# JJKK1313/DiTreeOnlinePlanner

Measured on AMD Instinct MI355X. Metric: candidate tree-expansions/sec (carmaze, H=32), higher is better.
Workload: dtype f16x3; 1 GPU; cfgs/carmaze.yaml + fm_policy flow sampler (K=1), batch=1024 candidates per GPU, H=32 (4 chunks x 8 steps), boxes.csv 20x20, 1024-node tree snapshot, seeded random weights; batch_per_gpu=1024, global_batch=1024, edge_length=32, action_horizon=8, pred_horizon=64, flow_steps=1, tree_nodes=1024, parallelism=candidates sharded x1

## Files before the change

ditreeonlineplanner_amd/csrc/conv_tiles.hip:

```cpp
#include <type_traits>

#include "denoise_device.h"

static thread_local bool g_dn_dry_run = false;
void denoise_set_dry_run(bool on) { g_dn_dry_run = on; }
bool denoise_dry_run() { return g_dn_dry_run; }

template <int PREC>
__device__ __forceinline__ void gemm_epilogue(const ConvGemmParams& p, f32x16_t (&acc)[2][4], char* smem, int tm, int tn,
                                              int tid, int lane, int r5, int h, int wm, int wn,
                                              long long out_extra_bytes = 0) {

  constexpr int ET = PREC == 2 ? 1 : 0;
  float satm = 0.0f;
  const int c_l = wn * 128 + 4 * r5;
  const int n0 = tn * 256 + c_l;
  const bool n_ok = n0 < p.N;
  float bias4[4] = {0.f, 0.f, 0.f, 0.f};
  if (p.bias != nullptr && n_ok) {
    f32x4_t t = *(const f32x4_t*)(p.bias + n0);
#pragma unroll
    for (int j = 0; j < 4; ++j) bias4[j] = t[j];
  }
#pragma unroll
  for (int mb = 0; mb < 2; ++mb)
#pragma unroll
    for (int j = 0; j < 4; ++j)
#pragma unroll
      for (int i = 0; i < 16; ++i) {
        if constexpr (PREC == 2) acc[mb][j][i] = fmaf(acc[mb][j][i], p.w_scale, bias4[j]);
        else acc[mb][j][i] += bias4[j];
      }

  int blk_b[4], blk_l[4];
#pragma unroll
  for (int blk = 0; blk < 4; ++blk) {
    const int m0 = tm * 256 + wm * 64 + (blk >> 1) * 32 + (blk & 1) * 16;
    const int b = m0 / p.L;
    blk_b[blk] = b;
    blk_l[blk] = m0 - b * p.L;
  }

  if (p.mode >= MODE_GN_MISH) {
    float* s_sum = (float*)smem;
    float* s_sq = s_sum + 64;
    if (tid < 128) s_sum[tid] = 0.0f;
    const f32x4_t gam = *(const f32x4_t*)(p.gamma + n0);
    const f32x4_t bet = *(const f32x4_t*)(p.beta + n0);
    f32x4_t film_s[4], film_b[4];
    if (p.mode == MODE_GN_MISH_FILM) {
#pragma unroll
      for (int blk = 0; blk < 4; ++blk) {
        const float* fr = p.film + (long long)blk_b[blk] * p.film_ld + p.film_off + n0;
        film_s[blk] = *(const f32x4_t*)fr;
        film_b[blk] = *(const f32x4_t*)(fr + p.N);
      }
    }
    short4_t resv[2][8];
    auto fetch_res = [&](int blk, short4_t (&dst)[8]) {
#pragma unroll
      for (int i = 0; i < 8; ++i) {
        const int rofs = (i & 3) + 8 * (i >> 2) + 4 * h;
        const long long rrow = (long long)blk_b[blk] * p.res_Lp + blk_l[blk] + rofs + p.res_off;
        dst[i] = *(const short4_t*)((const char*)p.Res + (rrow * p.ldres + n0) * 2);
      }
    };
    const bool res_bf16 = (PREC != 1) && p.mode == MODE_GN_MISH_RES;
    if (res_bf16) fetch_res(0, resv[0]);
    __syncthreads();
    const int spt = 256 / p.L;
    const int gi = c_l / p.group_ch;
    const bool wide = p.group_ch >= 128;
    int slot[4];
#pragma unroll
    for (int blk = 0; blk < 4; ++blk) slot[blk] = blk_b[blk] - tm * spt;
    const float inv_cnt = 1.0f / (float)(p.group_ch * p.L);
    const bool ordered = p.L >= 128 || (p.group_ch == 256 && p.L >= 32);
    const bool adder = lane == 0 || (!wide && lane == 16);
    const int ocell = ((wm * 2 + wn) * 4 + gi) * 2;
    auto put = [&](float* cell, float (&t)[4]) {
      if (ordered) {
        if (p.L >= 64) { t[0] = (t[0] + t[1]) + (t[2] + t[3]); t[2] = 0.0f; }
        else { t[0] += t[1]; t[2] += t[3]; }
        if (adder) { cell[ocell] = t[0]; cell[ocell + 1] = t[2]; }
      } else if (adder) {
#pragma unroll
        for (int blk = 0; blk < 4; ++blk) atomicAdd(&cell[slot[blk] * 4 + gi], t[blk]);
      }
    };
    auto get = [&](const float* cell, float (&t)[4]) {
      if (!ordered) {
#pragma unroll
        for (int blk = 0; blk < 4; ++blk) t[blk] = cell[slot[blk] * 4 + gi];
        return;
      }
#pragma unroll
      for (int blk = 0; blk < 4; blk += 2) {
        const int r0 = slot[blk] * p.L;
        const int w0 = r0 >> 6, nw = p.L >= 64 ? p.L >> 6 : 1, sub = (r0 >> 5) & 1;
        float v = 0.0f;
        for (int w = w0; w < w0 + nw; ++w) {
          v += cell[((w * 2 + 0) * 4 + gi) * 2 + sub];
          v += cell[((w * 2 + 1) * 4 + gi) * 2 + sub];
        }
        t[blk] = v; t[blk + 1] = v;
      }
    };
    float mean[4], rstd[4];
    if constexpr (PREC != 1) {
      float ps[4], pq[4];
#pragma unroll
      for (int blk = 0; blk < 4; ++blk) {
        float s = 0.f, q = 0.f;
#pragma unroll
        for (int j = 0; j < 4; ++j)
#pragma unroll
          for (int i = 0; i < 8; ++i) {
            const float v = acc[blk >> 1][j][(blk & 1) * 8 + i];
            s += v;
            q = fmaf(v, v, q);
          }
        s += __shfl_xor(s, 1); q += __shfl_xor(q, 1);
        s += __shfl_xor(s, 2); q += __shfl_xor(q, 2);
        s += __shfl_xor(s, 4); q += __shfl_xor(q, 4);
        s += __shfl_xor(s, 8); q += __shfl_xor(q, 8);
        s += __shfl_xor(s, 32); q += __shfl_xor(q, 32);
        if (wide) { s += __shfl_xor(s, 16); q += __shfl_xor(q, 16); }
        ps[blk] = s; pq[blk] = q;
      }
      put(s_sum, ps);
      put(s_sq, pq);
      __syncthreads();
      get(s_sum, ps);
      get(s_sq, pq);
#pragma unroll
      for (int blk = 0; blk < 4; ++blk) {
        mean[blk] = ps[blk] * inv_cnt;
        const float var = fmaxf(pq[blk] * inv_cnt - mean[blk] * mean[blk], 0.0f);
        rstd[blk] = rsqrtf(var + p.eps);
      }
    } else {
    {
      float ps[4];
#pragma unroll
      for (int blk = 0; blk < 4; ++blk) {
        float s = 0.f;
#pragma unroll
        for (int j = 0; j < 4; ++j)
#pragma unroll
          for (int i = 0; i < 8; ++i) s += acc[blk >> 1][j][(blk & 1) * 8 + i];
        ps[blk] = s;
      }
#pragma unroll
      for (int blk = 0; blk < 4; ++blk) {
        float s = ps[blk];
        s += __shfl_xor(s, 1); s += __shfl_xor(s, 2); s += __shfl_xor(s, 4); s += __shfl_xor(s, 8);
        s += __shfl_xor(s, 32);
        if (wide) s += __shfl_xor(s, 16);
        ps[blk] = s;
      }
      put(s_sum, ps);
      __syncthreads();
      get(s_sum, ps);
#pragma unroll
      for (int blk = 0; blk < 4; ++blk) mean[blk] = ps[blk] * inv_cnt;
    }
    {
      float ps[4];
#pragma unroll
      for (int blk = 0; blk < 4; ++blk) {
        float s = 0.f;
#pragma unroll
        for (int j = 0; j < 4; ++j)
#pragma unroll
          for (int i = 0; i < 8; ++i) {
            float d = acc[blk >> 1][j][(blk & 1) * 8 + i] - mean[blk];
            s += d * d;
          }
        s += __shfl_xor(s, 1); s += __shfl_xor(s, 2); s += __shfl_xor(s, 4); s += __shfl_xor(s, 8);
        s += __shfl_xor(s, 32);
        if (wide) s += __shfl_xor(s, 16);
        ps[blk] = s;
      }
      put(s_sq, ps);
      __syncthreads();
      get(s_sq, ps);
#pragma unroll
      for (int blk = 0; blk < 4; ++blk) rstd[blk] = rsqrtf(ps[blk] * inv_cnt + p.eps);
    }

    }

#pragma unroll
    for (int blk = 0; blk < 4; ++blk) {
      if (res_bf16 && blk < 3) fetch_res(blk + 1, resv[(blk + 1) & 1]);
      f32x4_t fs = {1.f, 1.f, 1.f, 1.f}, fb = {0.f, 0.f, 0.f, 0.f};
      if (p.mode == MODE_GN_MISH_FILM) { fs = film_s[blk]; fb = film_b[blk]; }
      float ga[4], be[4];
#pragma unroll
      for (int j = 0; j < 4; ++j) { ga[j] = gam[j] * rstd[blk]; be[j] = bet[j] - mean[blk] * ga[j]; }
#pragma unroll
      for (int i = 0; i < 8; ++i) {
        const int ii = (blk & 1) * 8 + i;
        const int rofs = (i & 3) + 8 * (i >> 2) + 4 * h;
        const int b = blk_b[blk], l = blk_l[blk] + rofs;
        float v[4];
#pragma unroll
        for (int j = 0; j < 4; ++j) v[j] = mish_f<PREC == 1 ? 1 : 0>(acc[blk >> 1][j][ii] * ga[j] + be[j]) * fs[j] + fb[j];
        if (p.mode == MODE_GN_MISH_RES) {
          if constexpr (PREC != 1) {
            const short4_t rv = resv[blk & 1][i];
#pragma unroll
            for (int j = 0; j < 4; ++j) v[j] += e2f<ET>((unsigned short)rv[j]);
          } else {
            const long long rrow = (long long)b * p.res_Lp + l + p.res_off;
            const f32x4_t rv = *(const f32x4_t*)((const char*)p.Res + (rrow * p.ldres + n0) * 4);
#pragma unroll
            for (int j = 0; j < 4; ++j) v[j] += rv[j];
          }
        }
        const long long orow = (long long)b * p.out_Lp + (long long)l * p.out_stride + p.out_off;
        const long long oidx = orow * p.ldc + p.out_coff + n0;
        if constexpr (PREC == 1) {
          const f32x4_t o = {v[0], v[1], v[2], v[3]};
          *(f32x4_t*)((char*)p.Out + out_extra_bytes + oidx * 4) = o;
        } else {
          short4_t o;
          if constexpr (ET == 1) { sat_see2(satm, v[0], v[1]); sat_see2(satm, v[2], v[3]); }
#pragma unroll
          for (int j = 0; j < 4; ++j) o[j] = (short)f2e<ET>(v[j]);
          *(short4_t*)((char*)p.Out + out_extra_bytes + oidx * 2) = o;
        }
      }
    }
    if constexpr (ET == 1) sat_flush(p.sat, satm);
    return;
  }

#pragma unroll
  for (int blk = 0; blk < 4; ++blk) {
#pragma unroll
    for (int i = 0; i < 8; ++i) {
      const int ii = (blk & 1) * 8 + i;
      const int rofs = (i & 3) + 8 * (i >> 2) + 4 * h;
      const int m = tm * 256 + wm * 64 + (blk >> 1) * 32 + (blk & 1) * 16 + rofs;
      if (m >= p.M || !n_ok) continue;
      int b = blk_b[blk], l = blk_l[blk] + rofs;
      if ((p.L & 15) != 0) { b = m / p.L; l = m - b * p.L; }
      const long long orow = (long long)b * p.out_Lp + (long long)l * p.out_stride + p.out_off;
      const long long oidx = orow * p.ldc + p.out_coff + n0;
      if (p.out_f32 || PREC == 1) {
        const f32x4_t o = {acc[blk >> 1][0][ii], acc[blk >> 1][1][ii], acc[blk >> 1][2][ii], acc[blk >> 1][3][ii]};
        *(f32x4_t*)((char*)p.Out + out_extra_bytes + oidx * 4) = o;
      } else {
        short4_t o;
        if constexpr (ET == 1) { sat_see2(satm, acc[blk >> 1][0][ii], acc[blk >> 1][1][ii]); sat_see2(satm, acc[blk >> 1][2][ii], acc[blk >> 1][3][ii]); }
#pragma unroll
        for (int j = 0; j < 4; ++j) o[j] = (short)f2e<ET>(acc[blk >> 1][j][ii]);
        *(short4_t*)((char*)p.Out + out_extra_bytes + oidx * 2) = o;
      }
    }
  }
  if constexpr (ET == 1) sat_flush(p.sat, satm);
}

template <int PREC, bool C2D = false>
__global__ void __launch_bounds__(512, 2) conv_gemm_kernel(ConvGemmParams p) {
  constexpr int ES = (PREC == 1) ? 4 : 2;
  constexpr int ET = PREC == 2 ? 1 : 0;
  constexpr int EK = 128 / ES;
  constexpr int EPS = 16 / ES;
  extern __shared__ __attribute__((aligned(16))) char smem[];

  const int tid = threadIdx.x, lane = tid & 63, w = tid >> 6;
  const int r5 = lane & 31, h = lane >> 5;
  const int wm = w >> 1, wn = w & 1;
  const int ntn = (p.N + 255) >> 8;
  const int ntm = (p.M + 255) >> 8;
  const int tile = xcd_remap(blockIdx.x, ntm * ntn);
  const int tm = tile / ntn, tn = tile - tm * ntn;
  const int K = p.taps * p.Cin;
  const int kpt = p.Cin / EK;
  int nk = K / EK;
  int k_first = 0;
  long long out_extra = 0;
  if constexpr (C2D) {
    if (p.splitk > 1) {
      const int per = (nk + p.splitk - 1) / p.splitk;
      k_first = blockIdx.y * per;
      nk = min(nk - k_first, per);
      out_extra = (long long)blockIdx.y * p.slab_stride * 4;
    }
  }

  const char* Abase = (const char*)p.A;
  const char* Wbase = (const char*)p.W;
  long long aoff[4], boff[4];
#pragma unroll
  for (int q = 0; q < 4; ++q) {
    const int r = (w * 4 + q) * 8 + (lane >> 3);
    const int sw = (r >> 1) & 7;
    const int slot = (lane & 7) ^ sw;
    int m = tm * 256 + r;
    m = m < p.M ? m : p.M - 1;
    const int b = m / p.L, l = m - b * p.L;
    aoff[q] = (((long long)b * p.in_Lp + (long long)l * p.in_stride + p.in_off) * p.lda + slot * EPS) * ES;
    const int c = (r & 128) + 4 * (r & 31) + ((r >> 5) & 3);
    boff[q] = (((long long)(tn * 256 + c)) * K + slot * EPS) * ES;
  }
  const char* pa[4];
  const char* pb[4];
#pragma unroll
  for (int q = 0; q < 4; ++q) {
    pa[q] = Abase + aoff[q];
    pb[q] = Wbase + boff[q] + (long long)k_first * 128;
  }
  int kin = C2D ? (k_first % kpt) : 0;
  const long long a_tap_jump = ((long long)p.lda - (long long)p.Cin + EK) * ES;
  const char* c2_base[4];
  int c2_ih0[4], c2_iw0[4], c2_slot[4];
  int c2_tap = C2D ? (k_first / kpt) : 0;
  if constexpr (C2D) {
#pragma unroll
    for (int q = 0; q < 4; ++q) {
      const int r = (w * 4 + q) * 8 + (lane >> 3);
      int m = tm * 256 + r;
      m = m < p.M ? m : p.M - 1;
      const int b = m / p.c2_OHW, rem = m - b * p.c2_OHW;
      const int oh = rem / p.c2_OW, ow = rem - oh * p.c2_OW;
      c2_base[q] = Abase + (long long)b * p.c2_H * p.c2_W * p.Cin * ES;
      c2_ih0[q] = oh * p.c2_stride - p.c2_pad;
      c2_iw0[q] = ow * p.c2_stride - p.c2_pad;
      c2_slot[q] = ((lane & 7) ^ ((r >> 1) & 7)) * 16;
    }
  }
  auto c2_point = [&]() {
    const int kh = p.c2_kh[c2_tap], kw = p.c2_kw[c2_tap];
#pragma unroll
    for (int q = 0; q < 4; ++q) {
      const int ih = c2_ih0[q] + kh, iw = c2_iw0[q] + kw;
      const bool ok = ih >= 0 && ih < p.c2_H && iw >= 0 && iw < p.c2_W;
      const char* src = c2_base[q] + ((long long)(ih * p.c2_W + iw) * p.Cin + kin * EK) * ES;
      pa[q] = (ok ? src : (const char*)p.zero) + c2_slot[q];
    }
  };
  if constexpr (C2D) c2_point();
  auto advance = [&]() {
    ++kin;
    if constexpr (C2D) {
      if (kin == kpt) { kin = 0; ++c2_tap; }
      if (c2_tap < p.taps) c2_point();
#pragma unroll
      for (int q = 0; q < 4; ++q) pb[q] += 128;
    } else {
      long long ainc = 128;
      if (kin == kpt) { kin = 0; ainc = a_tap_jump; }
#pragma unroll
      for (int q = 0; q < 4; ++q) {
        pa[q] += ainc;
        pb[q] += 128;
      }
    }
  };
  auto stage_piece = [&](int q, char* sbase) {
    if (q < 4)
      __builtin_amdgcn_global_load_lds((const GLOBAL_AS void*)pa[q], (LDS_AS void*)(sbase + (w * 4 + q) * 1024), 16, 0, 0);
    else
      __builtin_amdgcn_global_load_lds((const GLOBAL_AS void*)pb[q - 4],
                                       (LDS_AS void*)(sbase + 32768 + (w * 4 + q - 4) * 1024), 16, 0, 0);
  };

  f32x16_t acc[2][4];
#pragma unroll
  for (int mb = 0; mb < 2; ++mb)
#pragma unroll
    for (int j = 0; j < 4; ++j)
#pragma unroll
      for (int i = 0; i < 16; ++i) acc[mb][j][i] = 0.0f;

  const int swl = (r5 >> 1) & 7;
  const int a_row_off = (wm * 64 + r5) * 128;
  const int b_row_off = 32768 + (wn * 128 + r5) * 128;

  auto kstep = [&](const char* sb, auto stage_tag, char* snext) {
    constexpr bool STAGE = decltype(stage_tag)::value;
    if constexpr (PREC != 1) {
      short8_t af[2][2], bfr[2][4];
      auto rd = [&](int ks, int slot) {
        const int ps = (((ks << 1) | h) ^ swl) << 4;
#pragma unroll
        for (int mb = 0; mb < 2; ++mb)
          af[slot][mb] = *(const short8_t*)(sb + a_row_off + mb * 4096 + ps);
#pragma unroll
        for (int j = 0; j < 4; ++j)
          bfr[slot][j] = *(const short8_t*)(sb + b_row_off + j * 4096 + ps);
      };
      if constexpr (STAGE) {
#pragma unroll
        for (int q = 0; q < 8; ++q) stage_piece(q, snext);
      }
      rd(0, 0);
#pragma unroll
      for (int ks = 0; ks < 4; ++ks) {
        if (ks < 3) rd(ks + 1, (ks + 1) & 1);
#pragma unroll
        for (int mb = 0; mb < 2; ++mb)
#pragma unroll
          for (int j = 0; j < 4; ++j)
            acc[mb][j] = mfma32<ET>(af[ks & 1][mb], bfr[ks & 1][j], acc[mb][j]);
      }
      if constexpr (STAGE) __builtin_amdgcn_sched_group_barrier(0x020, 8, 0);
      __builtin_amdgcn_sched_group_barrier(0x100, 6, 0);
#pragma unroll
      for (int ks = 0; ks < 4; ++ks) {
        if (ks < 3) __builtin_amdgcn_sched_group_barrier(0x100, 6, 0);
        __builtin_amdgcn_sched_group_barrier(0x008, 8, 0);
      }
    } else {
#pragma unroll
      for (int sl = 0; sl < 8; ++sl) {
        const int ps = (sl ^ swl) << 4;
        f32x4_t af[2], bfr[4];
#pragma unroll
        for (int mb = 0; mb < 2; ++mb) af[mb] = *(const f32x4_t*)(sb + a_row_off + mb * 4096 + ps);
#pragma unroll
        for (int j = 0; j < 4; ++j) bfr[j] = *(const f32x4_t*)(sb + b_row_off + j * 4096 + ps);
#pragma unroll
        for (int s2 = 0; s2 < 2; ++s2) {
#pragma unroll
          for (int mb = 0; mb < 2; ++mb) {
            const float a = h ? af[mb][2 * s2 + 1] : af[mb][2 * s2];
#pragma unroll
            for (int j = 0; j < 4; ++j) {
              const float bv = h ? bfr[j][2 * s2 + 1] : bfr[j][2 * s2];
              acc[mb][j] = __builtin_amdgcn_mfma_f32_32x32x2f32(a, bv, acc[mb][j], 0, 0, 0);
            }
          }
        }
        if constexpr (STAGE) stage_piece(sl, snext);
      }
    }
  };

#pragma unroll
  for (int q = 0; q < 8; ++q) stage_piece(q, smem);
  advance();
  for (int kt = 0; kt < nk - 1; ++kt) {
    asm volatile("s_waitcnt vmcnt(0)" ::: "memory");
    __syncthreads();
    kstep(smem + (kt & 1) * 65536, std::true_type{}, smem + ((kt + 1) & 1) * 65536);
    advance();
  }
  asm volatile("s_waitcnt vmcnt(0)" ::: "memory");
  __syncthreads();
  kstep(smem + ((nk - 1) & 1) * 65536, std::false_type{}, nullptr);
  __syncthreads();
  gemm_epilogue<PREC>(p, acc, smem, tm, tn, tid, lane, r5, h, wm, wn, out_extra);
}

template <int ET, bool SPLIT, bool SHORT = false>
__device__ __forceinline__ void gemm_epilogue16(const ConvGemmParams& p, f32x4_t (&acc)[4][8], char* smem, int tm, int tn,
                                                int tid, int lane, int r4, int h4, int wm, int wn) {
  const int c_l = wn * 128 + 8 * r4;
  const int n0 = tn * 256 + c_l;
  {
    f32x4_t b0 = {0.f, 0.f, 0.f, 0.f}, b1 = b0;
    if (p.bias != nullptr) { b0 = *(const f32x4_t*)(p.bias + n0); b1 = *(const f32x4_t*)(p.bias + n0 + 4); }
    if constexpr (ET == 1) {
      const float ws = p.w_scale;
#pragma unroll
      for (int mb = 0; mb < 4; ++mb)
#pragma unroll
        for (int j = 0; j < 4; ++j) { acc[mb][j] = acc[mb][j] * ws + b0[j]; acc[mb][4 + j] = acc[mb][4 + j] * ws + b1[j]; }
    } else if (p.bias != nullptr) {
#pragma unroll
      for (int mb = 0; mb < 4; ++mb)
#pragma unroll
        for (int j = 0; j < 4; ++j) { acc[mb][j] += b0[j]; acc[mb][4 + j] += b1[j]; }
    }
  }
  constexpr bool short_l = SHORT;
  const int lane_b = short_l ? (4 * h4) / p.L : 0, lane_l = -lane_b * p.L;
  int blk_b[4], blk_l[4];
#pragma unroll
  for (int mb = 0; mb < 4; ++mb) {
    const int m0 = tm * 256 + wm * 64 + mb * 16;
    const int b = m0 / p.L;
    blk_b[mb] = b;
    blk_l[mb] = m0 - b * p.L;
  }
  auto store_row = [&](char* o, const float (&v)[8]) {
    short8_t hi, lo;
    if constexpr (ET == 1) {
      sat_check_row(p.sat, v);
#pragma unroll
      for (int jj = 0; jj < 4; ++jj) {
        const f32x2_t c = {__builtin_amdgcn_fmed3f(v[2 * jj], -65504.0f, 65504.0f),
                           __builtin_amdgcn_fmed3f(v[2 * jj + 1], -65504.0f, 65504.0f)};
        const half2_t h = __builtin_convertvector(c, half2_t);
        const short2_t hs = __builtin_bit_cast(short2_t, h);
        hi[2 * jj] = hs[0]; hi[2 * jj + 1] = hs[1];
        if constexpr (SPLIT) {
          const half2_t l = __builtin_convertvector(c - __builtin_convertvector(h, f32x2_t), half2_t);
          const short2_t ls = __builtin_bit_cast(short2_t, l);
          lo[2 * jj] = ls[0]; lo[2 * jj + 1] = ls[1];
        }
      }
    } else {
#pragma unroll
      for (int j = 0; j < 8; ++j) {
        hi[j] = (short)f2bf(v[j]);
        if constexpr (SPLIT) lo[j] = (short)f2bf(v[j] - bf2f((unsigned short)hi[j]));
      }
    }
    *(short8_t*)o = hi;
    if constexpr (SPLIT) *(short8_t*)(o + p.out_plane) = lo;
  };
  auto out_ptr = [&](int mb, int esize) {
    const long long orow = (long long)(blk_b[mb] + lane_b) * p.out_Lp + (long long)(blk_l[mb] + 4 * h4 + lane_l) * p.out_stride + p.out_off;
    return (char*)p.Out + (orow * p.ldc + p.out_coff + n0) * esize;
  };
  if (p.mode < MODE_GN_MISH) {
    const int esize = p.out_f32 ? 4 : 2;
    const long long ostep = (long long)p.out_stride * p.ldc * esize;
#pragma unroll
    for (int mb = 0; mb < 4; ++mb) {
      char* ob = out_ptr(mb, esize);
#pragma unroll
      for (int i = 0; i < 4; ++i, ob += ostep) {
        float v[8];
#pragma unroll
        for (int j = 0; j < 8; ++j) v[j] = acc[mb][j][i];
        if (p.out_f32) {
          *(f32x4_t*)ob = f32x4_t{v[0], v[1], v[2], v[3]};
          *(f32x4_t*)(ob + 16) = f32x4_t{v[4], v[5], v[6], v[7]};
        } else {
          store_row(ob, v);
        }
      }
    }
    return;
  }
  const bool has_film = p.mode == MODE_GN_MISH_FILM, has_res = p.mode == MODE_GN_MISH_RES;
  const int spt = 256 / p.L;
  const int ns = spt > 16 ? spt * 4 : 64;
  float* s_sum = (float*)smem;
  float* s_sq = s_sum + ns;
  float* s_gb = s_sq + ns;
  float* s_film = s_gb + 512;
  const bool film_direct = has_film && short_l;
  const int b_last = p.M / p.L - 1;
  for (int i = tid; i < 2 * ns; i += 512) s_sum[i] = 0.0f;
  s_gb[tid] = tid < 256 ? p.gamma[tn * 256 + tid] : p.beta[tn * 256 + tid - 256];
  if (has_film && !film_direct) {
    for (int idx = tid; idx < spt * 128; idx += 512) {
      const int sm = idx >> 7, c4 = idx & 127;
      const int b = min(tm * spt + sm, b_last);
      const float* src = p.film + (long long)b * p.film_ld + p.film_off + tn * 256 + (c4 & 63) * 4 + (c4 >> 6) * p.N;
      *(f32x4_t*)(s_film + sm * 512 + c4 * 4) = *(const f32x4_t*)src;
    }
  }
  f32x4_t rh[2], rl[2];
  const long long rstep = (long long)p.ldres * 2;
  auto fetch_film = [&](int mb) {
    const float* fr = p.film + (long long)min(blk_b[mb] + lane_b, b_last) * p.film_ld + p.film_off + n0;
    rh[0] = *(const f32x4_t*)fr; rh[1] = *(const f32x4_t*)(fr + 4);
    rl[0] = *(const f32x4_t*)(fr + p.N); rl[1] = *(const f32x4_t*)(fr + p.N + 4);
  };
  if (film_direct) fetch_film(0);
  auto fetch_res = [&](int r) {
    const long long rrow = (long long)(blk_b[r >> 2] + lane_b) * p.res_Lp + blk_l[r >> 2] + 4 * h4 + lane_l + p.res_off;
    const char* rp = (const char*)p.Res + (rrow * p.ldres + n0) * 2 + (r & 3) * rstep;
    rh[r & 1] = *(const f32x4_t*)rp;
    if constexpr (SPLIT) rl[r & 1] = *(const f32x4_t*)(rp + p.res_plane);
  };
  if (has_res) { fetch_res(0); fetch_res(1); }
  __syncthreads();
  const int gi = c_l / p.group_ch;
  const bool wide = p.group_ch >= 128;
  const float inv_cnt = 1.0f / (float)(p.group_ch * p.L);
  int slot[4];
#pragma unroll
  for (int mb = 0; mb < 4; ++mb) slot[mb] = (blk_b[mb] + lane_b - tm * spt) * 4 + gi;
  const bool ordered = !short_l && (p.L >= 128 || (p.group_ch == 256 && p.L >= 32));
  const int hsame = short_l ? (p.L == 8 ? 2 : 1) : 4;
  const bool adder = (r4 == 0 || (!wide && r4 == 8)) && (h4 & (hsame - 1)) == 0;
  const int ocell = ((wm * 2 + wn) * 4 + gi) * 2;
  auto block_sums = [&](float (&s)[4], float* cell) {
#pragma unroll
    for (int mb = 0; mb < 4; ++mb) s[mb] = dpp_add<0xB1>(s[mb]);
#pragma unroll
    for (int mb = 0; mb < 4; ++mb) s[mb] = dpp_add<0x4E>(s[mb]);
#pragma unroll
    for (int mb = 0; mb < 4; ++mb) s[mb] = dpp_add<0x141>(s[mb]);
    if (wide) {
#pragma unroll
      for (int mb = 0; mb < 4; ++mb) s[mb] = dpp_add<0x140>(s[mb]);
    }
    if (hsame >= 2) {
#pragma unroll
      for (int mb = 0; mb < 4; ++mb) s[mb] += __shfl_xor(s[mb], 16);
    }
    if (hsame == 4) {
#pragma unroll
      for (int mb = 0; mb < 4; ++mb) s[mb] += __shfl_xor(s[mb], 32);
    }
    if (ordered) {
      if (p.L >= 64) { s[0] = (s[0] + s[1]) + (s[2] + s[3]); s[2] = 0.0f; }
      else { s[0] += s[1]; s[2] += s[3]; }
      if (adder) { cell[ocell] = s[0]; cell[ocell + 1] = s[2]; }
    } else if (adder) {
#pragma unroll
      for (int mb = 0; mb < 4; ++mb) atomicAdd(&cell[slot[mb]], s[mb]);
    }
  };
  auto cell_sums = [&](const float* cell, float (&t)[4]) {
    if (!ordered) {
#pragma unroll
      for (int mb = 0; mb < 4; ++mb) t[mb] = cell[slot[mb]];
      return;
    }
#pragma unroll
    for (int mb = 0; mb < 4; mb += 2) {
      const int r0 = (blk_b[mb] - tm * spt) * p.L;
      const int w0 = r0 >> 6, nw = p.L >= 64 ? p.L >> 6 : 1, sub = (r0 >> 5) & 1;
      float v = 0.0f;
      for (int w = w0; w < w0 + nw; ++w) {
        v += cell[((w * 2 + 0) * 4 + gi) * 2 + sub];
        v += cell[((w * 2 + 1) * 4 + gi) * 2 + sub];
      }
      t[mb] = v; t[mb + 1] = v;
    }
  };
  float mean_[4], rstd_[4];
  auto pair = [&](int mb, int j, int ip) { return f32x2_t{acc[mb][j][2 * ip], acc[mb][j][2 * ip + 1]}; };
  if constexpr (!SPLIT) {
    float s[4], q[4];
#pragma unroll
    for (int mb = 0; mb < 4; ++mb) {
      f32x2_t s2 = {0.f, 0.f}, q2 = {0.f, 0.f};
#pragma unroll
      for (int j = 0; j < 8; ++j)
#pragma unroll
        for (int ip = 0; ip < 2; ++ip) {
          const f32x2_t v = pair(mb, j, ip);
          s2 += v;
          q2 = __builtin_elementwise_fma(v, v, q2);
        }
      s[mb] = s2[0] + s2[1];
      q[mb] = q2[0] + q2[1];
    }
    block_sums(s, s_sum);
    block_sums(q, s_sq);
    __syncthreads();
    cell_sums(s_sum, s);
    cell_sums(s_sq, q);
#pragma unroll
    for (int mb = 0; mb < 4; ++mb) {
      mean_[mb] = s[mb] * inv_cnt;
      const float var = fmaxf(q[mb] * inv_cnt - mean_[mb] * mean_[mb], 0.0f);
      rstd_[mb] = rsqrtf(var + p.eps);
    }
  } else {
    float s[4];
#pragma unroll
    for (int mb = 0; mb < 4; ++mb) {
      f32x2_t s2 = {0.f, 0.f};
#pragma unroll
      for (int j = 0; j < 8; ++j)
#pragma unroll
        for (int ip = 0; ip < 2; ++ip) s2 += pair(mb, j, ip);
      s[mb] = s2[0] + s2[1];
    }
    block_sums(s, s_sum);
    __syncthreads();
    cell_sums(s_sum, s);
#pragma unroll
    for (int mb = 0; mb < 4; ++mb) {
      mean_[mb] = s[mb] * inv_cnt;
      f32x2_t q2 = {0.f, 0.f};
#pragma unroll
      for (int j = 0; j < 8; ++j) {
#pragma unroll
        for (int ip = 0; ip < 2; ++ip) {
          const f32x2_t d = pair(mb, j, ip) - mean_[mb];
          q2 = __builtin_elementwise_fma(d, d, q2);
        }
        if (j & 1) __builtin_amdgcn_sched_barrier(0);
      }
      s[mb] = q2[0] + q2[1];
    }
    block_sums(s, s_sq);
    __syncthreads();
    cell_sums(s_sq, s);
#pragma unroll
    for (int mb = 0; mb < 4; ++mb) rstd_[mb] = rsqrtf(s[mb] * inv_cnt + p.eps);
  }
  const long long ostep = (long long)p.out_stride * p.ldc * 2;
#pragma unroll
  for (int mb = 0; mb < 4; ++mb) {
    float mean = mean_[mb];
    const float rstd = rstd_[mb];
    if constexpr (SPLIT) asm volatile("" : "+v"(mean));
    float ga[8], be[8], fs[8], fb[8];
    {
      const f32x4_t gam0 = *(const f32x4_t*)(s_gb + c_l), gam1 = *(const f32x4_t*)(s_gb + c_l + 4);
      const f32x4_t bet0 = *(const f32x4_t*)(s_gb + 256 + c_l), bet1 = *(const f32x4_t*)(s_gb + 256 + c_l + 4);
#pragma unroll
      for (int j = 0; j < 4; ++j) {
        ga[j] = gam0[j] * rstd; ga[4 + j] = gam1[j] * rstd;
        if constexpr (SPLIT) { be[j] = bet0[j]; be[4 + j] = bet1[j]; }
        else { be[j] = bet0[j] - mean * ga[j]; be[4 + j] = bet1[j] - mean * ga[4 + j]; }
      }
    }
    if (film_direct) {
#pragma unroll
      for (int j = 0; j < 4; ++j) { fs[j] = rh[0][j]; fs[4 + j] = rh[1][j]; fb[j] = rl[0][j]; fb[4 + j] = rl[1][j]; }
      if (mb + 1 < 4) fetch_film(mb + 1);
    } else if (has_film) {
      const float* fr = s_film + (blk_b[mb] - tm * spt) * 512 + c_l;
      const f32x4_t f0 = *(const f32x4_t*)fr, f1 = *(const f32x4_t*)(fr + 4);
      const f32x4_t f2 = *(const f32x4_t*)(fr + 256), f3 = *(const f32x4_t*)(fr + 260);
#pragma unroll
      for (int j = 0; j < 4; ++j) { fs[j] = f0[j]; fs[4 + j] = f1[j]; fb[j] = f2[j]; fb[4 + j] = f3[j]; }
    }
    char* ob = out_ptr(mb, 2);
#pragma unroll
    for (int ip = 0; ip < 2; ++ip, ob += 2 * ostep) {
      const int r = mb * 4 + 2 * ip;
      f32x2_t v[8];
      if (has_res) {
        const short8_t h0 = __builtin_bit_cast(short8_t, rh[0]), h1 = __builtin_bit_cast(short8_t, rh[1]);
#pragma unroll
        for (int j = 0; j < 8; ++j) v[j] = f32x2_t{e2f<ET>((unsigned short)h0[j]), e2f<ET>((unsigned short)h1[j])};
        if constexpr (SPLIT) {
          const short8_t l0 = __builtin_bit_cast(short8_t, rl[0]), l1 = __builtin_bit_cast(short8_t, rl[1]);
#pragma unroll
          for (int j = 0; j < 8; ++j) v[j] += f32x2_t{e2f<ET>((unsigned short)l0[j]), e2f<ET>((unsigned short)l1[j])};
        }
        if (r + 2 < 16) { fetch_res(r + 2); fetch_res(r + 3); }
      } else {
#pragma unroll
        for (int j = 0; j < 8; ++j) v[j] = f32x2_t{0.f, 0.f};
      }
#pragma unroll
      for (int j = 0; j < 8; ++j) {
        f32x2_t x = pair(mb, j, ip);
        if constexpr (SPLIT) x = (x - mean) * ga[j] + be[j];
        else x = x * ga[j] + be[j];
        x = mish2<SPLIT ? 2 : 0>(x);
        v[j] += x;
      }
      if (has_film) {
#pragma unroll
        for (int j = 0; j < 8; ++j) v[j] = v[j] * fs[j] + fb[j];
      }
      float row[8];
#pragma unroll
      for (int j = 0; j < 8; ++j) row[j] = v[j][0];
      store_row(ob, row);
#pragma unroll
      for (int j = 0; j < 8; ++j) row[j] = v[j][1];
      store_row(ob + ostep, row);
      __builtin_amdgcn_sched_barrier(0);
    }
  }
}

template <int ET>
__device__ __forceinline__ void mm16_snake(f32x4_t (&acc)[4][8], const short8_t (&a)[4], const short8_t (&b)[4], int half) {
#pragma unroll
  for (int mb = 0; mb < 4; ++mb)
#pragma unroll
    for (int jj = 0; jj < 4; ++jj) {
      const int j = (mb & 1) ? 3 - jj : jj;
      acc[mb][half * 4 + j] = mfma16<ET>(a[mb], b[j], acc[mb][half * 4 + j]);
    }
}

#ifdef HALO16_STAMP
__device__ unsigned long long g_halo_stamp[8];
extern "C" int ditree_debug_halo_stamp(unsigned long long* out) {
  return (int)hipMemcpyFromSymbol(out, HIP_SYMBOL(g_halo_stamp), sizeof(g_halo_stamp));
}
__device__ unsigned int g_x3_phase[8][32];
extern "C" int ditree_debug_x3_phase(unsigned int* out) {
  return (int)hipMemcpyFromSymbol(out, HIP_SYMBOL(g_x3_phase), sizeof(g_x3_phase));
}
#define X3_STAMP_MAX 65536
__device__ unsigned long long g_x3_stamp[X3_STAMP_MAX][6];
__device__ unsigned int g_x3_count;
extern "C" int ditree_debug_x3_stamp(unsigned long long* out, unsigned int* count, int reset) {
  int rc = (int)hipMemcpyFromSymbol(count, HIP_SYMBOL(g_x3_count), 4);
  if (rc == 0 && out != nullptr) rc = (int)hipMemcpyFromSymbol(out, HIP_SYMBOL(g_x3_stamp), sizeof(unsigned long long) * 6 * X3_STAMP_MAX);
  if (rc == 0 && reset) { unsigned int z = 0; rc = (int)hipMemcpyToSymbol(HIP_SYMBOL(g_x3_count), &z, 4); }
  return rc;
}
#endif
template <int ET>
__global__ void __launch_bounds__(512, 2) conv3_halo16_kernel(ConvGemmParams p) {
  extern __shared__ __attribute__((aligned(16))) char smem[];
  constexpr int A_BUF = 40960, W_BUF = 32768, W_BASE = 2 * A_BUF;
  const int tid = threadIdx.x, lane = tid & 63;
  const int w = __builtin_amdgcn_readfirstlane(tid >> 6);
  const int r4 = lane & 15, h4 = lane >> 4;
  const int wm = w >> 1, wn = w & 1;
  const int ntn = (p.N + 255) >> 8;
  const int ntm = (p.M + 255) >> 8;
  const int tile = xcd_remap_strips(blockIdx.x, ntm, ntn, p.xcd_strips);
  const int tm = tile / ntn, tn = tile - tm * ntn;
  const int L = p.L, Lp = p.in_Lp, S = 256 / L;
  const int a_rows = S * Lp;
  const int nc = p.Cin >> 6;
  const long long K = 3LL * p.Cin;

  unsigned pa0, pa4, pb;
  const char* const a_base = (const char*)p.A + ((long long)tm * S * Lp + p.in_off) * p.lda * 2;
  const char* const w_base = (const char*)p.W + ((long long)tn * 256) * K * 2;
  const __amdgpu_buffer_rsrc_t a_rsrc = __builtin_amdgcn_make_buffer_rsrc((void*)a_base, 0, 0x7fffffff, 0x00020000);
  const __amdgpu_buffer_rsrc_t w_rsrc = __builtin_amdgcn_make_buffer_rsrc((void*)w_base, 0, 0x7fffffff, 0x00020000);
  {
    const int r = w * 8 + (lane >> 3);
    const int slot = (lane & 7) ^ (r & 7);
    pa0 = (unsigned)((r * p.lda + slot * 8) * 2);
    const int r4r = r + 256;
    const int rs = r4r < a_rows ? r4r : a_rows - 1;
    pa4 = (unsigned)((rs * p.lda + slot * 8) * 2);
  }
  const int a_piece = 64 * p.lda * 2;
  long long wq[4];
  {
    const int lr = lane >> 3;
    const int slot = (lane & 7) ^ lr;
    pb = (unsigned)(((long long)(8 * lr) * K + slot * 8) * 2);
#pragma unroll
    for (int q = 0; q < 4; ++q) {
      const int r0 = (w * 4 + q) * 8;
      const int cu = (r0 & 128) + 8 * (r0 & 8) + ((r0 >> 4) & 7);
      wq[q] = (long long)cu * K * 2;
    }
  }
  const int w_tap = p.Cin * 2;
  auto issue_a = [&](int c, int i) {
    __builtin_amdgcn_raw_ptr_buffer_load_lds(a_rsrc, (LDS_AS void*)(smem + (c & 1) * A_BUF + (w + 8 * i) * 1024), 16,
                                             i < 4 ? pa0 : pa4, c * 128 + (i < 4 ? i * a_piece : 0), 0, 0);
  };
  auto issue_w = [&](int c, int t, int q) {
    __builtin_amdgcn_raw_ptr_buffer_load_lds(w_rsrc, (LDS_AS void*)(smem + W_BASE + ((c + t) & 1) * W_BUF + (w * 4 + q) * 1024),
                                             16, pb, (int)wq[q] + c * 128 + t * w_tap, 0, 0);
  };

  int lrow0;
  {
    const int ml = wm * 64 + r4;
    const int sb = ml / L;
    lrow0 = sb * Lp + (ml - sb * L);
  }
  int lstep[4];
#pragma unroll
  for (int mb = 0; mb < 4; ++mb) lstep[mb] = 16 * mb + 2 * (((wm * 64 + 16 * mb) / L) - ((wm * 64) / L));
  const int swl = r4 & 7;
  const int b_row_off = (wn * 128 + r4) * 128;

  f32x4_t acc[4][8];
#pragma unroll
  for (int mb = 0; mb < 4; ++mb)
#pragma unroll
    for (int j = 0; j < 8; ++j) acc[mb][j] = f32x4_t{0.f, 0.f, 0.f, 0.f};

  short8_t af[2][4], bq[2][4];
  auto rdA = [&](int set, int c, int t, int ks) {
    const char* ab = smem + (c & 1) * A_BUF;
#pragma unroll
    for (int mb = 0; mb < 4; ++mb) {
      const int row = lrow0 + lstep[mb] + t;
      const int ps = (((ks << 2) | h4) ^ (row & 7)) << 4;
      af[set][mb] = *(const short8_t*)(ab + row * 128 + ps);
    }
  };
  auto rdB = [&](int set, int c, int t, int ks, int half) {
    const char* wb = smem + W_BASE + ((c + t) & 1) * W_BUF + b_row_off + half * 8192;
    const int psb = (((ks << 2) | h4) ^ swl) << 4;
#pragma unroll
    for (int jj = 0; jj < 4; ++jj) bq[set][jj] = *(const short8_t*)(wb + jj * 2048 + psb);
  };
  auto mm = [&](int aset, int bset, int half, int mb, int jj) {
    acc[mb][half * 4 + jj] = mfma16<ET>(af[aset][mb], bq[bset][jj], acc[mb][half * 4 + jj]);
  };
  auto mm16 = [&](int aset, int bset, int half) { mm16_snake<ET>(acc, af[aset], bq[bset], half); };

  auto step = [&](auto tT, auto tNext, auto tIW, auto tIA, auto tVM, int c) {
    constexpr int T = decltype(tT)::value;
    constexpr bool HAS_NEXT = decltype(tNext)::value, ISSUE_W = decltype(tIW)::value, ISSUE_A = decltype(tIA)::value;
    constexpr int VM = decltype(tVM)::value;
    constexpr int NV = ISSUE_W ? 4 : 0;
    asm volatile("" : "+v"(lrow0));
    __builtin_amdgcn_s_setprio(2);
    rdB(1, c, T, 0, 1);
    mm16(0, 0, 0);
    __builtin_amdgcn_sched_group_barrier(0x100, 4, 0);
    __builtin_amdgcn_sched_group_barrier(0x008, 16, 0);
    __builtin_amdgcn_sched_barrier(0);
    __builtin_amdgcn_s_setprio(1);
    rdA(1, c, T, 1);
    rdB(0, c, T, 1, 0);
    mm16(0, 1, 1);
    __builtin_amdgcn_sched_group_barrier(0x100, 8, 0);
    __builtin_amdgcn_sched_group_barrier(0x008, 16, 0);
    __builtin_amdgcn_sched_barrier(0);
    __builtin_amdgcn_s_setprio(0);
    rdB(1, c, T, 1, 1);
    mm16(1, 0, 0);
    if constexpr (ISSUE_A && T != 2) {
      if constexpr (T == 0) { issue_a(c + 1, 0); issue_a(c + 1, 1); issue_a(c + 1, 2); }
      else { issue_a(c + 1, 3); issue_a(c + 1, 4); }
      __builtin_amdgcn_sched_group_barrier(0x100, 4, 0);
      __builtin_amdgcn_sched_group_barrier(0x008, 4, 0);
      __builtin_amdgcn_sched_group_barrier(0x020, 1, 0);
      __builtin_amdgcn_sched_group_barrier(0x008, 4, 0);
      __builtin_amdgcn_sched_group_barrier(0x020, 1, 0);
      __builtin_amdgcn_sched_group_barrier(0x008, 4, 0);
      if constexpr (T == 0) __builtin_amdgcn_sched_group_barrier(0x020, 1, 0);
      __builtin_amdgcn_sched_group_barrier(0x008, 4, 0);
    } else {
      __builtin_amdgcn_sched_group_barrier(0x100, 4, 0);
      __builtin_amdgcn_sched_group_barrier(0x008, 16, 0);
    }
    __builtin_amdgcn_sched_barrier(0);
    if constexpr (HAS_NEXT) {
      if constexpr (VM == 0) asm volatile("s_waitcnt vmcnt(0) lgkmcnt(0)" ::: "memory");
      else if constexpr (VM == 3) asm volatile("s_waitcnt vmcnt(3) lgkmcnt(0)" ::: "memory");
      else asm volatile("s_waitcnt vmcnt(2) lgkmcnt(0)" ::: "memory");
      __builtin_amdgcn_s_barrier();
      __builtin_amdgcn_s_setprio(3);
      constexpr int T1 = (T + 1) % 3;
      rdA(0, c + (T + 1) / 3, T1, 0);
      rdB(0, c + (T + 1) / 3, T1, 0, 0);
    }
    constexpr int T2 = (T + 2) % 3;
    const int c2 = c + (T + 2) / 3;
#pragma unroll
    for (int mb = 0; mb < 4; ++mb)
#pragma unroll
      for (int jj = 0; jj < 4; ++jj) {
        mm(1, 1, 1, mb, (mb & 1) ? 3 - jj : jj);
        const int i = mb * 4 + jj;
        const int d = (i & 1) ? -1 : (i >> 1);
        if constexpr (ISSUE_W) { if (d >= 0 && d < 4) issue_w(c2, T2, d); }
      }
    if constexpr (HAS_NEXT) __builtin_amdgcn_sched_group_barrier(0x100, 8, 1);
#pragma unroll
    for (int i = 0; i < 16; ++i) {
      __builtin_amdgcn_sched_group_barrier(0x008, 1, 1);
      if (!(i & 1) && (i >> 1) < NV) __builtin_amdgcn_sched_group_barrier(0x020, 1, 1);
    }
    __builtin_amdgcn_sched_barrier(0);
  };
  using I0 = std::integral_constant<int, 0>;
  using I1 = std::integral_constant<int, 1>;
  using I2 = std::integral_constant<int, 2>;
  using I3 = std::integral_constant<int, 3>;
  using Tt = std::true_type;
  using Ff = std::false_type;

#pragma unroll
  for (int i = 0; i < 5; ++i) issue_a(0, i);
#pragma unroll
  for (int q = 0; q < 4; ++q) issue_w(0, 0, q);
  asm volatile("s_waitcnt vmcnt(0)" ::: "memory");
  __builtin_amdgcn_s_barrier();
#pragma unroll
  for (int q = 0; q < 4; ++q) issue_w(0, 1, q);
  rdA(0, 0, 0, 0);
  rdB(0, 0, 0, 0, 0);

#ifdef HALO16_STAMP
  const unsigned long long st0 = __builtin_amdgcn_s_memtime(), rt0 = __builtin_amdgcn_s_memrealtime();
#endif
  for (int c = 0; c < nc - 2; ++c) {
    step(I0{}, Tt{}, Tt{}, Tt{}, I3{}, c);
    step(I1{}, Tt{}, Tt{}, Tt{}, I2{}, c);
    step(I2{}, Tt{}, Tt{}, Tt{}, I0{}, c);
  }
#ifdef HALO16_STAMP
  if (blockIdx.x == 100 && tid == 0 && nc >= 32) {
    g_halo_stamp[0] = __builtin_amdgcn_s_memtime() - st0;
    g_halo_stamp[1] = __builtin_amdgcn_s_memrealtime() - rt0;
    g_halo_stamp[2] = (unsigned long long)(nc - 2) * 3;
  }
#endif
  {
    const int c = nc - 2;
    step(I0{}, Tt{}, Tt{}, Tt{}, I0{}, c);
    step(I1{}, Tt{}, Tt{}, Tt{}, I0{}, c);
    step(I2{}, Tt{}, Tt{}, Ff{}, I0{}, c);
  }
  {
    const int c = nc - 1;
    step(I0{}, Tt{}, Tt{}, Ff{}, I0{}, c);
    step(I1{}, Tt{}, Ff{}, Ff{}, I0{}, c);
    step(I2{}, Ff{}, Ff{}, Ff{}, I0{}, c);
  }
  __builtin_amdgcn_s_setprio(0);
  __syncthreads();
  gemm_epilogue16<ET, false>(p, acc, smem, tm, tn, tid, lane, r4, h4, wm, wn);
}

template <int ET, bool SHORT = false, bool SPLITK = false, int NP = 5>
__global__ void __launch_bounds__(512, 2) conv3_halo16x3_kernel(ConvGemmParams p) {
  extern __shared__ __attribute__((aligned(16))) char smem[];
  static_assert(NP == 5 || NP == 6, "five or six activation pieces");
  constexpr int A_BUF = NP * 8192, W_BUF = 32768, W_BASE = 2 * A_BUF;
  const int tid = threadIdx.x, lane = tid & 63;
  const int w = __builtin_amdgcn_readfirstlane(tid >> 6);
  const int r4 = lane & 15, h4 = lane >> 4;
  const int wm = w >> 1, wn = w & 1;
  const int ntn = (p.N + 255) >> 8;
  const int ntm = (p.M + 255) >> 8;
  const int tile = xcd_remap_strips(blockIdx.x, ntm, ntn, p.xcd_strips);
  const int tm = tile / ntn, tn = tile - tm * ntn;
  const int L = p.L, Lp = p.in_Lp, S = 256 / L;
  const int a_rows = S * Lp;
  const int nv_all = p.Cin >> 5;
  const int v_lo = SPLITK ? (int)blockIdx.y * (nv_all / p.splitk) : 0;
  const int nv = SPLITK ? v_lo + nv_all / p.splitk : nv_all;
  const long long K = 3LL * p.Cin;
  const unsigned a_plane = (unsigned)p.a_plane, w_plane = (unsigned)p.w_plane;

  unsigned pa0, pa4, pa5 = 0, pb;
  const char* const a_base = (const char*)p.A + ((long long)tm * S * Lp + p.in_off) * p.lda * 2;
  const char* const w_base = (const char*)p.W + ((long long)tn * 256) * K * 2;
  const __amdgpu_buffer_rsrc_t a_rsrc = __builtin_amdgcn_make_buffer_rsrc((void*)a_base, 0, 0x7fffffff, 0x00020000);
  const __amdgpu_buffer_rsrc_t w_rsrc = __builtin_amdgcn_make_buffer_rsrc((void*)w_base, 0, 0x7fffffff, 0x00020000);
  {
    const int r = w * 8 + (lane >> 3);
    const int slot = (lane & 7) ^ (r & 7);
    const unsigned po = (slot & 4) ? a_plane : 0u;
    pa0 = (unsigned)((r * p.lda + (slot & 3) * 8) * 2) + po;
    const int r4r = r + 256;
    const int rs = r4r < a_rows ? r4r : a_rows - 1;
    pa4 = (unsigned)((rs * p.lda + (slot & 3) * 8) * 2) + po;
    if constexpr (NP == 6) {
      const int r5r = r + 320;
      const int rs5 = r5r < a_rows ? r5r : a_rows - 1;
      pa5 = (unsigned)((rs5 * p.lda + (slot & 3) * 8) * 2) + po;
    }
  }
  const int a_piece = 64 * p.lda * 2;
  long long wq[4];
  {
    const int lr = lane >> 3;
    const int slot = (lane & 7) ^ lr;
    pb = (unsigned)(((long long)(8 * lr) * K + (slot & 3) * 8) * 2) + ((slot & 4) ? w_plane : 0u);
#pragma unroll
    for (int q = 0; q < 4; ++q) {
      const int r0 = (w * 4 + q) * 8;
      const int cu = (r0 & 128) + 8 * (r0 & 8) + ((r0 >> 4) & 7);
      wq[q] = (long long)cu * K * 2;
    }
  }
  const int w_tap = p.Cin * 2;
  auto issue_a = [&](int v, int i) {
    __builtin_amdgcn_raw_ptr_buffer_load_lds(a_rsrc, (LDS_AS void*)(smem + (v & 1) * A_BUF + (w + 8 * i) * 1024), 16,
                                             i < 4 ? pa0 : (i == 4 ? pa4 : pa5), v * 64 + (i < 4 ? i * a_piece : 0), 0, 0);
  };
  auto issue_w = [&](int v, int t, int q) {
    __builtin_amdgcn_raw_ptr_buffer_load_lds(w_rsrc, (LDS_AS void*)(smem + W_BASE + ((v + t) & 1) * W_BUF + (w * 4 + q) * 1024),
                                             16, pb, (int)wq[q] + v * 64 + t * w_tap, 0, 0);
  };

  int lrow0;
  {
    const int ml = wm * 64 + r4;
    const int sb = ml / L;
    lrow0 = sb * Lp + (ml - sb * L);
  }
  int lstep[4];
#pragma unroll
  for (int mb = 0; mb < 4; ++mb) lstep[mb] = 16 * mb + 2 * (((wm * 64 + 16 * mb) / L) - ((wm * 64) / L));
  const int swl = r4 & 7;
  const int b_row_off = (wn * 128 + r4) * 128;

  f32x4_t acc[4][8];
#pragma unroll
  for (int mb = 0; mb < 4; ++mb)
#pragma unroll
    for (int j = 0; j < 8; ++j) acc[mb][j] = f32x4_t{0.f, 0.f, 0.f, 0.f};

  short8_t af[2][4], bq[2][4];
  auto rdA = [&](int set, int v, int t, int pl) {
    const char* ab = smem + (v & 1) * A_BUF;
#pragma unroll
    for (int mb = 0; mb < 4; ++mb) {
      const int row = lrow0 + lstep[mb] + t;
      const int ps = (((pl << 2) | h4) ^ (row & 7)) << 4;
      af[set][mb] = *(const short8_t*)(ab + row * 128 + ps);
    }
  };
  auto rdB = [&](int set, int v, int t, int pl, int half) {
    const char* wb = smem + W_BASE + ((v + t) & 1) * W_BUF + b_row_off + half * 8192;
    const int psb = (((pl << 2) | h4) ^ swl) << 4;
#pragma unroll
    for (int jj = 0; jj < 4; ++jj) bq[set][jj] = *(const short8_t*)(wb + jj * 2048 + psb);
  };
  auto mm = [&](int aset, int bset, int half, int mb, int jj) {
    acc[mb][half * 4 + jj] = mfma16<ET>(af[aset][mb], bq[bset][jj], acc[mb][half * 4 + jj]);
  };
  auto mm16 = [&](int aset, int bset, int half) { mm16_snake<ET>(acc, af[aset], bq[bset], half); };

#ifdef X3_PHASE_STAMP
  unsigned pst[24];
#define PSTAMP(k) do { pst[T * 8 + (k)] = (unsigned)__builtin_amdgcn_s_memtime(); __builtin_amdgcn_sched_barrier(0); } while (0)
#else
#define PSTAMP(k) do { } while (0)
#endif
  auto step = [&](auto tT, auto tNext, auto tIW, auto tIA, auto tVM, int v) {
    constexpr int T = decltype(tT)::value;
    constexpr bool HAS_NEXT = decltype(tNext)::value, ISSUE_W = decltype(tIW)::value, ISSUE_A = decltype(tIA)::value;
    constexpr int VM = decltype(tVM)::value;
    asm volatile("" : "+v"(lrow0));
    PSTAMP(0);
    __builtin_amdgcn_s_setprio(2);
    rdB(1, v, T, 1, 1);
    mm16(0, 0, 0);
    __builtin_amdgcn_sched_group_barrier(0x100, 4, 0);
    __builtin_amdgcn_sched_group_barrier(0x008, 16, 0);
    __builtin_amdgcn_sched_barrier(0);
    PSTAMP(1);
    rdB(0, v, T, 0, 0);
    rdA(1, v, T, 1);
    mm16(0, 1, 1);
    __builtin_amdgcn_sched_group_barrier(0x100, 8, 0);
    __builtin_amdgcn_sched_group_barrier(0x008, 16, 0);
    __builtin_amdgcn_sched_barrier(0);
    PSTAMP(2);
    __builtin_amdgcn_s_setprio(1);
    rdB(1, v, T, 0, 1);
    mm16(0, 0, 0);
    __builtin_amdgcn_sched_group_barrier(0x100, 4, 0);
    __builtin_amdgcn_sched_group_barrier(0x008, 16, 0);
    __builtin_amdgcn_sched_barrier(0);
    PSTAMP(3);
    mm16(1, 0, 0);
    if constexpr (ISSUE_A && T != 2) {
      if constexpr (T == 0) { issue_a(v + 1, 0); issue_a(v + 1, 1); issue_a(v + 1, 2); }
      else { issue_a(v + 1, 3); issue_a(v + 1, 4); if constexpr (NP == 6) issue_a(v + 1, 5); }
      __builtin_amdgcn_sched_group_barrier(0x008, 4, 2);
      __builtin_amdgcn_sched_group_barrier(0x020, 1, 2);
      __builtin_amdgcn_sched_group_barrier(0x008, 4, 2);
      __builtin_amdgcn_sched_group_barrier(0x020, 1, 2);
      __builtin_amdgcn_sched_group_barrier(0x008, 4, 2);
      if constexpr (T == 0 || NP == 6) __builtin_amdgcn_sched_group_barrier(0x020, 1, 2);
      __builtin_amdgcn_sched_group_barrier(0x008, 4, 2);
    }
    __builtin_amdgcn_sched_barrier(0);
    PSTAMP(4);
    __builtin_amdgcn_s_setprio(0);
    mm16(0, 1, 1);
    __builtin_amdgcn_sched_barrier(0);
    PSTAMP(5);
    if constexpr (HAS_NEXT) {
      if constexpr (VM == 0) asm volatile("s_waitcnt vmcnt(0) lgkmcnt(0)" ::: "memory");
      else if constexpr (VM == 3) asm volatile("s_waitcnt vmcnt(3) lgkmcnt(0)" ::: "memory");
      else asm volatile("s_waitcnt vmcnt(2) lgkmcnt(0)" ::: "memory");
      __builtin_amdgcn_s_barrier();
      __builtin_amdgcn_s_setprio(3);
      PSTAMP(6);
      constexpr int T1 = (T + 1) % 3;
      rdA(0, v + (T + 1) / 3, T1, 0);
      rdB(0, v + (T + 1) / 3, T1, 1, 0);
    }
    constexpr int T2 = (T + 2) % 3;
    const int v2 = v + (T + 2) / 3;
#pragma unroll
    for (int mb = 0; mb < 4; ++mb)
#pragma unroll
      for (int jj = 0; jj < 4; ++jj) {
        mm(1, 1, 1, mb, (mb & 1) ? 3 - jj : jj);
        const int i = mb * 4 + jj;
        const int d = (i & 1) ? -1 : (i >> 1);
        if constexpr (ISSUE_W) { if (d >= 0 && d < 4) issue_w(v2, T2, d); }
      }
    if constexpr (HAS_NEXT) __builtin_amdgcn_sched_group_barrier(0x100, 8, 1);
    constexpr int NV = ISSUE_W ? 4 : 0;
#pragma unroll
    for (int i = 0; i < 16; ++i) {
      __builtin_amdgcn_sched_group_barrier(0x008, 1, 1);
      if (!(i & 1) && (i >> 1) < NV) __builtin_amdgcn_sched_group_barrier(0x020, 1, 1);
    }
    __builtin_amdgcn_sched_barrier(0);
    PSTAMP(7);
  };
#undef PSTAMP
  using I0 = std::integral_constant<int, 0>;
  using I1 = std::integral_constant<int, 1>;
  using I2 = std::integral_constant<int, 2>;
  using I3 = std::integral_constant<int, 3>;
  using Tt = std::true_type;
  using Ff = std::false_type;

#ifdef HALO16_STAMP
  const unsigned long long xs0 = __builtin_amdgcn_s_memrealtime();
#endif
#pragma unroll
  for (int i = 0; i < NP; ++i) issue_a(v_lo, i);
#pragma unroll
  for (int q = 0; q < 4; ++q) issue_w(v_lo, 0, q);
  asm volatile("s_waitcnt vmcnt(0)" ::: "memory");
  __builtin_amdgcn_s_barrier();
#pragma unroll
  for (int q = 0; q < 4; ++q) issue_w(v_lo, 1, q);
  rdA(0, v_lo, 0, 0);
  rdB(0, v_lo, 0, 1, 0);
#ifdef HALO16_STAMP
  const unsigned long long xs1 = __builtin_amdgcn_s_memrealtime();
#endif

  using IT1 = std::integral_constant<int, NP == 6 ? 3 : 2>;
  for (int v = v_lo; v < nv - 2; ++v) {
    step(I0{}, Tt{}, Tt{}, Tt{}, I3{}, v);
    step(I1{}, Tt{}, Tt{}, Tt{}, IT1{}, v);
    step(I2{}, Tt{}, Tt{}, Tt{}, I0{}, v);
  }
#ifdef X3_PHASE_STAMP
  if (blockIdx.x == 100 && lane == 0 && nv == 64) {
#pragma unroll
    for (int k = 0; k < 24; ++k) g_x3_phase[w][k] = pst[k];
    g_x3_phase[w][24] = (unsigned)nv;
  }
#endif
  {
    const int v = nv - 2;
    step(I0{}, Tt{}, Tt{}, Tt{}, I0{}, v);
    step(I1{}, Tt{}, Tt{}, Tt{}, I0{}, v);
    step(I2{}, Tt{}, Tt{}, Ff{}, I0{}, v);
  }
  {
    const int v = nv - 1;
    step(I0{}, Tt{}, Tt{}, Ff{}, I0{}, v);
    step(I1{}, Tt{}, Ff{}, Ff{}, I0{}, v);
    step(I2{}, Ff{}, Ff{}, Ff{}, I0{}, v);
  }
  __builtin_amdgcn_s_setprio(0);
  __syncthreads();
#ifdef HALO16_STAMP
  const unsigned long long xs2 = __builtin_amdgcn_s_memrealtime();
#endif
  if constexpr (SPLITK) {
    const int ntiles = ntm * ntn;
    float* mine = p.sk_ws + ((size_t)blockIdx.y * ntiles + tile) * 65536;
#pragma unroll
    for (int mb = 0; mb < 4; ++mb)
#pragma unroll
      for (int j = 0; j < 8; ++j) *(f32x4_t*)(mine + ((mb * 8 + j) * 512 + tid) * 4) = acc[mb][j];
    __threadfence();
    __syncthreads();
    int* s_last = (int*)smem;
    if (tid == 0) *s_last = atomicAdd(p.sk_cnt + tile, 1) == p.splitk - 1;
    __syncthreads();
    const bool last = *s_last != 0;
    __syncthreads();
    if (!last) return;
    __threadfence();
#pragma unroll
    for (int mb = 0; mb < 4; ++mb)
#pragma unroll
      for (int j = 0; j < 8; ++j) acc[mb][j] = f32x4_t{0.f, 0.f, 0.f, 0.f};
    for (int sp = 0; sp < p.splitk; ++sp) {
      const float* sl = p.sk_ws + ((size_t)sp * ntiles + tile) * 65536;
#pragma unroll
      for (int mb = 0; mb < 4; ++mb)
#pragma unroll
        for (int j = 0; j < 8; ++j) acc[mb][j] += *(const f32x4_t*)(sl + ((mb * 8 + j) * 512 + tid) * 4);
    }
    if (tid == 0) p.sk_cnt[tile] = 0;
  }
  gemm_epilogue16<ET, true, SHORT>(p, acc, smem, tm, tn, tid, lane, r4, h4, wm, wn);
#ifdef HALO16_STAMP
  __syncthreads();
  if (tid == 0) {
    const unsigned long long xs3 = __builtin_amdgcn_s_memrealtime();
    const unsigned int k = atomicAdd(&g_x3_count, 1u);
    if (k < X3_STAMP_MAX) {
      g_x3_stamp[k][0] = xs0; g_x3_stamp[k][1] = xs1; g_x3_stamp[k][2] = xs2; g_x3_stamp[k][3] = xs3;
      g_x3_stamp[k][4] = ((unsigned long long)nv << 32) | blockIdx.x;
      g_x3_stamp[k][5] = ((unsigned long long)__builtin_amdgcn_s_getreg((31 << 11) | 20) << 32) |
                         (unsigned int)__builtin_amdgcn_s_getreg((31 << 11) | 4);
    }
  }
#endif
}

template <int ET, bool SPLIT>
__global__ void __launch_bounds__(256) conv2d_small_kernel(ConvGemmParams p) {
  extern __shared__ __attribute__((aligned(16))) char smem[];
  constexpr int STAGE = 16384;
  constexpr int CK = SPLIT ? 32 : 64;
  const int tid = threadIdx.x, lane = tid & 63;
  const int w = __builtin_amdgcn_readfirstlane(tid >> 6);
  const int r5 = lane & 31, h = lane >> 5;
  const int wm = w >> 1, wn = w & 1;
  const int ntn = p.N >> 6;
  const int tm = blockIdx.x / ntn, tn = blockIdx.x - tm * ntn;
  const int kpt = p.Cin / CK;
  const long long K = (long long)p.taps * p.Cin;
  int k0 = 0, nk = p.taps * kpt;
  long long out_extra = 0;
  if (p.splitk > 1) {
    const int per = (nk + p.splitk - 1) / p.splitk;
    k0 = blockIdx.y * per;
    nk = min(nk - k0, per);
    out_extra = (long long)blockIdx.y * p.slab_stride;
  }

  const char* a_base[2];
  int ih0[2], iw0[2];
  const char* w_src[2];
  int slot_b[2];
  long long plane_a[2];
#pragma unroll
  for (int q = 0; q < 2; ++q) {
    const int r = (2 * w + q) * 8 + (lane >> 3);
    const int slot = (lane & 7) ^ ((r >> 1) & 7);
    slot_b[q] = SPLIT ? (slot & 3) * 16 : slot * 16;
    plane_a[q] = (SPLIT && (slot & 4)) ? p.a_plane : 0;
    const long long plane_w = (SPLIT && (slot & 4)) ? p.w_plane : 0;
    int m = tm * 64 + r;
    m = m < p.M ? m : p.M - 1;
    const int b = m / p.c2_OHW, rem = m - b * p.c2_OHW;
    const int oh = rem / p.c2_OW, ow = rem - oh * p.c2_OW;
    a_base[q] = (const char*)p.A + (long long)b * p.c2_H * p.c2_W * p.Cin * 2;
    ih0[q] = oh * p.c2_stride - p.c2_pad;
    iw0[q] = ow * p.c2_stride - p.c2_pad;
    w_src[q] = (const char*)p.W + ((long long)(tn * 64 + r) * K) * 2 + slot_b[q] + plane_w;
  }
  auto issue = [&](int kl) {
    const int k = k0 + kl;
    const int tap = k / kpt, kin = k - tap * kpt;
    const int kh = p.c2_kh[tap], kw = p.c2_kw[tap];
    char* st = smem + (kl % 3) * STAGE;
#pragma unroll
    for (int q = 0; q < 2; ++q) {
      const int ih = ih0[q] + kh, iw = iw0[q] + kw;
      const bool ok = ih >= 0 && ih < p.c2_H && iw >= 0 && iw < p.c2_W;
      const char* src = ok ? a_base[q] + ((long long)(ih * p.c2_W + iw) * p.Cin + kin * CK) * 2 + plane_a[q] : (const char*)p.zero;
      __builtin_amdgcn_global_load_lds((const GLOBAL_AS void*)(src + slot_b[q]), (LDS_AS void*)(st + (2 * w + q) * 1024), 16, 0, 0);
    }
#pragma unroll
    for (int q = 0; q < 2; ++q)
      __builtin_amdgcn_global_load_lds((const GLOBAL_AS void*)(w_src[q] + (long long)k * (CK * 2)),
                                       (LDS_AS void*)(st + 8192 + (2 * w + q) * 1024), 16, 0, 0);
  };

  f32x16_t acc;
#pragma unroll
  for (int i = 0; i < 16; ++i) acc[i] = 0.0f;
  const int a_row = wm * 32 + r5, b_row = wn * 32 + r5;
  const int a_off = a_row * 128, b_off = 8192 + b_row * 128;
  const int sa = (a_row >> 1) & 7, sb = (b_row >> 1) & 7;

  issue(0);
  if (nk > 1) issue(1);
  for (int k = 0; k < nk; ++k) {
    if (k + 1 < nk) asm volatile("s_waitcnt vmcnt(4)" ::: "memory");
    else asm volatile("s_waitcnt vmcnt(0)" ::: "memory");
    __builtin_amdgcn_s_barrier();
    if (k + 2 < nk) issue(k + 2);
    const char* st = smem + (k % 3) * STAGE;
    if constexpr (SPLIT) {
      short8_t af[4], bf[4];
#pragma unroll
      for (int ks = 0; ks < 4; ++ks) {
        af[ks] = *(const short8_t*)(st + a_off + ((((ks << 1) | h) ^ sa) << 4));
        bf[ks] = *(const short8_t*)(st + b_off + ((((ks << 1) | h) ^ sb) << 4));
      }
#pragma unroll
      for (int kk = 0; kk < 2; ++kk) acc = mfma32<ET>(af[kk], bf[kk + 2], acc);
#pragma unroll
      for (int kk = 0; kk < 2; ++kk) acc = mfma32<ET>(af[kk], bf[kk], acc);
#pragma unroll
      for (int kk = 0; kk < 2; ++kk) acc = mfma32<ET>(af[kk + 2], bf[kk], acc);
    } else {
#pragma unroll
      for (int ks = 0; ks < 4; ++ks) {
        const short8_t af = *(const short8_t*)(st + a_off + ((((ks << 1) | h) ^ sa) << 4));
        const short8_t bf = *(const short8_t*)(st + b_off + ((((ks << 1) | h) ^ sb) << 4));
        acc = mfma32<ET>(af, bf, acc);
      }
    }
    asm volatile("s_waitcnt lgkmcnt(0)" ::: "memory");
  }

  const int n = tn * 64 + wn * 32 + r5;
  float bias = (p.bias != nullptr && k0 == 0) ? p.bias[n] : 0.0f;
#pragma unroll
  for (int i = 0; i < 16; ++i) {
    const int m = tm * 64 + wm * 32 + (i & 3) + 8 * (i >> 2) + 4 * h;
    if (m < p.M) ((float*)p.Out)[out_extra + (long long)m * p.ldc + p.out_coff + n] = (ET == 1 ? acc[i] * p.w_scale : acc[i]) + bias;
  }
}

template <int ET, bool SPLIT, bool SHORT = false>
__global__ void __launch_bounds__(512, 2) gemm16_kernel(ConvGemmParams p) {
  extern __shared__ __attribute__((aligned(16))) char smem[];
  constexpr int BUF = 32768, W_BASE = 2 * BUF;
  const int tid = threadIdx.x, lane = tid & 63;
  const int w = __builtin_amdgcn_readfirstlane(tid >> 6);
  const int r4 = lane & 15, h4 = lane >> 4;
  const int wm = w >> 1, wn = w & 1;
  const int ntn = p.N >> 8, ntm = p.M >> 8;
  const int tile = xcd_remap_strips(blockIdx.x, ntm, ntn, p.xcd_strips);
  const int tm = tile / ntn, tn = tile - tm * ntn;
  constexpr int KB = SPLIT ? 64 : 128;
  const int nc = SPLIT ? (p.Cin >> 5) : (p.Cin >> 6), nk = p.taps * nc;
  const unsigned a_plane = (unsigned)p.a_plane, w_plane = (unsigned)p.w_plane;
  const long long K = (long long)p.taps * p.Cin;

  long long a_tile0;
  {
    const int m0 = tm * 256;
    const int b0 = m0 / p.L, l0 = m0 - b0 * p.L;
    a_tile0 = (((long long)b0 * p.in_Lp + (long long)l0 * p.in_stride + p.in_off) * p.lda) * 2;
  }
  const __amdgpu_buffer_rsrc_t a_rsrc =
      __builtin_amdgcn_make_buffer_rsrc((void*)((const char*)p.A + a_tile0), 0, 0x7fffffff, 0x00020000);
  const __amdgpu_buffer_rsrc_t w_rsrc =
      __builtin_amdgcn_make_buffer_rsrc((void*)((const char*)p.W + ((long long)tn * 256) * K * 2), 0, 0x7fffffff, 0x00020000);
  unsigned pae, pao, pbe, pbo;
  int aq[4], wq[4];
  {
    const int lr = lane >> 3;
    const int slot0 = (lane & 7) ^ (lr >> 1), slot1 = slot0 ^ 4;
    const int lrb = lr / p.L, lro = lrb * p.in_Lp + (lr - lrb * p.L) * p.in_stride;
    if constexpr (SPLIT) {
      pae = (unsigned)((lro * p.lda + (slot0 & 3) * 8) * 2) + ((slot0 & 4) ? a_plane : 0u);
      pao = (unsigned)((lro * p.lda + (slot1 & 3) * 8) * 2) + ((slot1 & 4) ? a_plane : 0u);
      pbe = (unsigned)(((long long)(8 * lr) * K + (slot0 & 3) * 8) * 2) + ((slot0 & 4) ? w_plane : 0u);
      pbo = (unsigned)(((long long)(8 * lr) * K + (slot1 & 3) * 8) * 2) + ((slot1 & 4) ? w_plane : 0u);
    } else {
      pae = (unsigned)((lro * p.lda + slot0 * 8) * 2);
      pao = (unsigned)((lro * p.lda + slot1 * 8) * 2);
      pbe = (unsigned)(((long long)(8 * lr) * K + slot0 * 8) * 2);
      pbo = (unsigned)(((long long)(8 * lr) * K + slot1 * 8) * 2);
    }
#pragma unroll
    for (int q = 0; q < 4; ++q) {
      const int r0 = (w * 4 + q) * 8;
      const int m = tm * 256 + r0;
      const int b = m / p.L, l = m - b * p.L;
      aq[q] = (int)((((long long)b * p.in_Lp + (long long)l * p.in_stride + p.in_off) * p.lda) * 2 - a_tile0);
      const int cu = (r0 & 128) + 8 * (r0 & 8) + ((r0 >> 4) & 7);
      wq[q] = (int)((long long)cu * K * 2);
    }
  }
  const int tap_bytes = p.lda * 2;
  auto src_off = [&](int k, int& ao, int& wo) {
    const int t = k / nc, c = k - t * nc;
    ao = t * tap_bytes + c * KB;
    wo = k * KB;
  };
  auto issue = [&](int kv) {
    int ao, wo;
    src_off(kv, ao, wo);
    char* ab = smem + (kv & 1) * BUF;
    char* wb = smem + W_BASE + (kv & 1) * BUF;
#pragma unroll
    for (int q = 0; q < 4; ++q)
      __builtin_amdgcn_raw_ptr_buffer_load_lds(a_rsrc, (LDS_AS void*)(ab + (w * 4 + q) * 1024), 16, (q & 1) ? pao : pae,
                                               aq[q] + ao, 0, 0);
#pragma unroll
    for (int q = 0; q < 4; ++q)
      __builtin_amdgcn_raw_ptr_buffer_load_lds(w_rsrc, (LDS_AS void*)(wb + (w * 4 + q) * 1024), 16, (q & 1) ? pbo : pbe,
                                               wq[q] + wo, 0, 0);
  };

  auto issue_wq = [&](int kv, int q) {
    int ao, wo;
    src_off(kv, ao, wo);
    __builtin_amdgcn_raw_ptr_buffer_load_lds(w_rsrc, (LDS_AS void*)(smem + W_BASE + (kv & 1) * BUF + (w * 4 + q) * 1024), 16,
                                             (q & 1) ? pbo : pbe, wq[q] + wo, 0, 0);
  };
  const int a_row = wm * 64 + r4;
  const int swa = (a_row >> 1) & 7;
  const int a_off = a_row * 128, b_off = (wn * 128 + r4) * 128;
  const int swb = (r4 >> 1) & 7;

  f32x4_t acc[4][8];
#pragma unroll
  for (int mb = 0; mb < 4; ++mb)
#pragma unroll
    for (int j = 0; j < 8; ++j) acc[mb][j] = f32x4_t{0.f, 0.f, 0.f, 0.f};
  short8_t af[2][4], bq[2][4];
  auto rdA = [&](int set, int k, int ks) {
    const char* ab = smem + (k & 1) * BUF + a_off + ((((ks << 2) | h4) ^ swa) << 4);
#pragma unroll
    for (int mb = 0; mb < 4; ++mb) af[set][mb] = *(const short8_t*)(ab + mb * 2048);
  };
  auto rdB = [&](int set, int k, int ks, int half) {
    const char* wb = smem + W_BASE + (k & 1) * BUF + b_off + half * 8192 + ((((ks << 2) | h4) ^ swb) << 4);
#pragma unroll
    for (int jj = 0; jj < 4; ++jj) bq[set][jj] = *(const short8_t*)(wb + jj * 2048);
  };
  auto mm = [&](int aset, int bset, int half, int mb, int jj) {
    acc[mb][half * 4 + jj] = mfma16<ET>(af[aset][mb], bq[bset][jj], acc[mb][half * 4 + jj]);
  };
  auto mm16 = [&](int aset, int bset, int half) {
#pragma unroll
    for (int mb = 0; mb < 4; ++mb)
#pragma unroll
      for (int jj = 0; jj < 4; ++jj) mm(aset, bset, half, mb, (mb & 1) ? 3 - jj : jj);
  };
  auto step = [&](auto tNext, auto tIssue, int k) {
    constexpr bool HAS_NEXT = decltype(tNext)::value, ISSUE = decltype(tIssue)::value;
    if constexpr (SPLIT) {
      rdB(1, k, 1, 1);
      mm16(0, 0, 0);
      if constexpr (HAS_NEXT) {
        issue_wq(k + 1, 0); issue_wq(k + 1, 1);
        __builtin_amdgcn_sched_group_barrier(0x100, 4, 0);
        __builtin_amdgcn_sched_group_barrier(0x008, 4, 0);
        __builtin_amdgcn_sched_group_barrier(0x020, 1, 0);
        __builtin_amdgcn_sched_group_barrier(0x008, 4, 0);
        __builtin_amdgcn_sched_group_barrier(0x020, 1, 0);
        __builtin_amdgcn_sched_group_barrier(0x008, 8, 0);
      } else
      {
      __builtin_amdgcn_sched_group_barrier(0x100, 4, 0);
      __builtin_amdgcn_sched_group_barrier(0x008, 16, 0);
      }
      __builtin_amdgcn_sched_barrier(0);
      rdB(0, k, 0, 0);
      rdA(1, k, 1);
      mm16(0, 1, 1);
      if constexpr (HAS_NEXT) {
        issue_wq(k + 1, 2); issue_wq(k + 1, 3);
        __builtin_amdgcn_sched_group_barrier(0x100, 8, 0);
        __builtin_amdgcn_sched_group_barrier(0x008, 4, 0);
        __builtin_amdgcn_sched_group_barrier(0x020, 1, 0);
        __builtin_amdgcn_sched_group_barrier(0x008, 4, 0);
        __builtin_amdgcn_sched_group_barrier(0x020, 1, 0);
        __builtin_amdgcn_sched_group_barrier(0x008, 8, 0);
      } else
      {
      __builtin_amdgcn_sched_group_barrier(0x100, 8, 0);
      __builtin_amdgcn_sched_group_barrier(0x008, 16, 0);
      }
      __builtin_amdgcn_sched_barrier(0);
      rdB(1, k, 0, 1);
      mm16(0, 0, 0);
      __builtin_amdgcn_sched_group_barrier(0x100, 4, 0);
      __builtin_amdgcn_sched_group_barrier(0x008, 16, 0);
      __builtin_amdgcn_sched_barrier(0);
      mm16(1, 0, 0);
      __builtin_amdgcn_sched_barrier(0);
      mm16(0, 1, 1);
      __builtin_amdgcn_sched_barrier(0);
    } else {
      rdB(1, k, 0, 1);
      mm16(0, 0, 0);
      __builtin_amdgcn_sched_group_barrier(0x100, 4, 0);
      __builtin_amdgcn_sched_group_barrier(0x008, 16, 0);
      __builtin_amdgcn_sched_barrier(0);
      rdA(1, k, 1);
      rdB(0, k, 1, 0);
      mm16(0, 1, 1);
      __builtin_amdgcn_sched_group_barrier(0x100, 8, 0);
      __builtin_amdgcn_sched_group_barrier(0x008, 16, 0);
      __builtin_amdgcn_sched_barrier(0);
      rdB(1, k, 1, 1);
      mm16(1, 0, 0);
      __builtin_amdgcn_sched_group_barrier(0x100, 4, 0);
      __builtin_amdgcn_sched_group_barrier(0x008, 16, 0);
      __builtin_amdgcn_sched_barrier(0);
    }
    int ao2 = 0, wo2 = 0;
    if constexpr (ISSUE) src_off(k + 2, ao2, wo2);
    if constexpr (HAS_NEXT) {
      asm volatile("s_waitcnt vmcnt(0) lgkmcnt(0)" ::: "memory");
      __builtin_amdgcn_s_barrier();
      rdA(0, k + 1, 0);
      rdB(0, k + 1, SPLIT ? 1 : 0, 0);
    }
#pragma unroll
    for (int mb = 0; mb < 4; ++mb)
#pragma unroll
      for (int jj = 0; jj < 4; ++jj) {
        mm(1, 1, 1, mb, (mb & 1) ? 3 - jj : jj);
        if constexpr (ISSUE) {
          const int m = mb * 4 + jj, i = (m & 1) ? -1 : (m >> 1);
          if (i >= 0 && i < 4)
            __builtin_amdgcn_raw_ptr_buffer_load_lds(a_rsrc, (LDS_AS void*)(smem + (k & 1) * BUF + (w * 4 + i) * 1024), 16,
                                                     (i & 1) ? pao : pae, aq[i] + ao2, 0, 0);
          else if (!SPLIT && i >= 4 && i < 8)
            __builtin_amdgcn_raw_ptr_buffer_load_lds(w_rsrc, (LDS_AS void*)(smem + W_BASE + (k & 1) * BUF + (w * 4 + i - 4) * 1024),
                                                     16, ((i - 4) & 1) ? pbo : pbe, wq[i - 4] + wo2, 0, 0);
        }
      }
    if constexpr (HAS_NEXT) __builtin_amdgcn_sched_group_barrier(0x100, 8, 1);
#pragma unroll
    for (int i = 0; i < 16; ++i) {
      __builtin_amdgcn_sched_group_barrier(0x008, 1, 1);
      if (ISSUE && !(i & 1) && (!SPLIT || i < 8)) __builtin_amdgcn_sched_group_barrier(0x020, 1, 1);
    }
    __builtin_amdgcn_sched_barrier(0);
  };
  using Tt = std::true_type;
  using Ff = std::false_type;

  issue(0);
  asm volatile("s_waitcnt vmcnt(0)" ::: "memory");
  __builtin_amdgcn_s_barrier();
  if (nk > 1) {
    if constexpr (SPLIT) {
      int ao, wo;
      src_off(1, ao, wo);
#pragma unroll
      for (int q = 0; q < 4; ++q)
        __builtin_amdgcn_raw_ptr_buffer_load_lds(a_rsrc, (LDS_AS void*)(smem + BUF + (w * 4 + q) * 1024), 16, (q & 1) ? pao : pae,
                                                 aq[q] + ao, 0, 0);
    } else {
      issue(1);
    }
  }
  rdA(0, 0, 0);
  rdB(0, 0, SPLIT ? 1 : 0, 0);
  for (int k = 0; k < nk - 2; ++k) step(Tt{}, Tt{}, k);
  if (nk >= 2) step(Tt{}, Ff{}, nk - 2);
  step(Ff{}, Ff{}, nk - 1);
  __syncthreads();
  gemm_epilogue16<ET, SPLIT, SHORT>(p, acc, smem, tm, tn, tid, lane, r4, h4, wm, wn);
}
enum { TILE_HALO, TILE_GEMM16, TILE_C2D_SMALL, TILE_GENERIC };
enum { TV_SPLIT = 1,
       TV_SHORT = 2,
       TV_SPLITK = 4,
       TV_NP6 = 8,
       TV_C2D = 16 };
struct TileVariant {
  void (*kernel)(ConvGemmParams);
  unsigned lds_bytes;
  unsigned block;
  int family, st;
  unsigned flags;
  int kind;
};
static const TileVariant k_tiles[] = {
    {conv3_halo16_kernel<0>, 147456, 512, TILE_HALO, ST_BF16, 0, 0},
    {conv3_halo16_kernel<1>, 147456, 512, TILE_HALO, ST_F16, 0, 0},
    {conv3_halo16x3_kernel<0>, 147456, 512, TILE_HALO, ST_BF16, TV_SPLIT, 0},
    {conv3_halo16x3_kernel<1>, 147456, 512, TILE_HALO, ST_F16, TV_SPLIT, 0},
    {conv3_halo16x3_kernel<0, true>, 147456, 512, TILE_HALO, ST_BF16, TV_SPLIT | TV_SHORT, 0},
    {conv3_halo16x3_kernel<1, true>, 147456, 512, TILE_HALO, ST_F16, TV_SPLIT | TV_SHORT, 0},
    {conv3_halo16x3_kernel<0, false, true>, 147456, 512, TILE_HALO, ST_BF16, TV_SPLIT | TV_SPLITK, 0},
    {conv3_halo16x3_kernel<1, false, true>, 147456, 512, TILE_HALO, ST_F16, TV_SPLIT | TV_SPLITK, 0},
    {conv3_halo16x3_kernel<0, true, true>, 147456, 512, TILE_HALO, ST_BF16, TV_SPLIT | TV_SHORT | TV_SPLITK, 0},
    {conv3_halo16x3_kernel<1, true, true>, 147456, 512, TILE_HALO, ST_F16, TV_SPLIT | TV_SHORT | TV_SPLITK, 0},
    {conv3_halo16x3_kernel<0, true, false, 6>, 163840, 512, TILE_HALO, ST_BF16, TV_SPLIT | TV_SHORT | TV_NP6, 0},
    {conv3_halo16x3_kernel<1, true, false, 6>, 163840, 512, TILE_HALO, ST_F16, TV_SPLIT | TV_SHORT | TV_NP6, 0},
    {gemm16_kernel<0, false>, 131072, 512, TILE_GEMM16, ST_BF16, 0, 1},
    {gemm16_kernel<1, false>, 131072, 512, TILE_GEMM16, ST_F16, 0, 1},
    {gemm16_kernel<0, true>, 131072, 512, TILE_GEMM16, ST_BF16, TV_SPLIT, 1},
    {gemm16_kernel<1, true>, 131072, 512, TILE_GEMM16, ST_F16, TV_SPLIT, 1},
    {gemm16_kernel<0, false, true>, 131072, 512, TILE_GEMM16, ST_BF16, TV_SHORT, 1},
    {gemm16_kernel<1, false, true>, 131072, 512, TILE_GEMM16, ST_F16, TV_SHORT, 1},
    {gemm16_kernel<0, true, true>, 131072, 512, TILE_GEMM16, ST_BF16, TV_SPLIT | TV_SHORT, 1},
    {gemm16_kernel<1, true, true>, 131072, 512, TILE_GEMM16, ST_F16, TV_SPLIT | TV_SHORT, 1},
    {conv2d_small_kernel<0, false>, 3 * 16384, 256, TILE_C2D_SMALL, ST_BF16, TV_C2D, 2},
    {conv2d_small_kernel<1, false>, 3 * 16384, 256, TILE_C2D_SMALL, ST_F16, TV_C2D, 2},
    {conv2d_small_kernel<0, true>, 3 * 16384, 256, TILE_C2D_SMALL, ST_BF16, TV_C2D | TV_SPLIT, 2},
    {conv2d_small_kernel<1, true>, 3 * 16384, 256, TILE_C2D_SMALL, ST_F16, TV_C2D | TV_SPLIT, 2},
    {conv_gemm_kernel<0, false>, 131072, 512, TILE_GENERIC, ST_BF16, 0, 1},
    {conv_gemm_kernel<1, false>, 131072, 512, TILE_GENERIC, ST_F32, 0, 1},
    {conv_gemm_kernel<2, false>, 131072, 512, TILE_GENERIC, ST_F16, 0, 1},
    {conv_gemm_kernel<0, true>, 131072, 512, TILE_GENERIC, ST_BF16, TV_C2D, 2},
    {conv_gemm_kernel<1, true>, 131072, 512, TILE_GENERIC, ST_F32, TV_C2D, 2},
    {conv_gemm_kernel<2, true>, 131072, 512, TILE_GENERIC, ST_F16, TV_C2D, 2},
};
static const TileVariant* find_tile(int family, int st, unsigned flags) {
  for (const TileVariant& v : k_tiles)
    if (v.family == family && v.st == st && v.flags == flags) return &v;
  return nullptr;
}

static const TileVariant* pick_tile(const ConvGemmParams& p, int fmt) {
  const int st = fmt_st(fmt);
  const bool split = fmt_split(fmt);
  const unsigned fsplit = split ? TV_SPLIT : 0;
  const bool tile16 = st != ST_F32 && !p.c2d && (p.M & 255) == 0 && (p.N & 255) == 0 && (p.Cin & 63) == 0;
  const bool l_ok = p.L >= 16 || (p.L == 8 && split) || (p.L == 4 && split && p.splitk <= 1);
  if (tile16 && p.taps == 3 && p.in_stride == 1 && p.in_Lp == p.L + 2 && (256 % p.L) == 0 && l_ok && p.Cin >= 192) {
    if (!split) return find_tile(TILE_HALO, st, 0);
    const unsigned fshort = p.L <= 8 ? TV_SHORT : 0;
    if (p.splitk > 1) return find_tile(TILE_HALO, st, TV_SPLIT | fshort | TV_SPLITK);
    return find_tile(TILE_HALO, st, TV_SPLIT | fshort | (p.L == 4 ? TV_NP6 : 0));
  }
  const bool short_l = p.L == 8 || p.L == 4;
  if (tile16 && (!p.out_f32 || p.mode == MODE_BIAS) && p.taps >= 1 && p.taps <= 3 && ((p.L & 15) == 0 || short_l) && p.M > 0 &&
      (p.mode == MODE_BIAS || (256 % p.L) == 0))
    return find_tile(TILE_GEMM16, st, fsplit | ((p.L & 15) != 0 ? TV_SHORT : 0));
  if (p.c2d && conv2d_small_eligible(fmt) && (p.N & 63) == 0 && (p.Cin & 63) == 0 && p.out_f32 && p.mode == MODE_BIAS)
    return find_tile(TILE_C2D_SMALL, st, TV_C2D | fsplit);
  if (split) return nullptr;
  return find_tile(TILE_GENERIC, st, p.c2d ? TV_C2D : 0);
}
bool conv2d_small_eligible(int fmt) { return fmt_st(fmt) != ST_F32; }
int conv_gemm_kind(const ConvGemmParams& p, int fmt) {
  const TileVariant* v = pick_tile(p, fmt);
  return v != nullptr ? v->kind : (p.c2d ? 2 : 1);
}
bool conv_gemm_supported(const ConvGemmParams& p, int fmt) { return pick_tile(p, fmt) != nullptr; }

static void ensure_lds_attrs() {
  static bool done[64] = {};
  int dev = 0;
  hipGetDevice(&dev);
  if (dev < 0 || dev >= 64 || done[dev]) return;
  done[dev] = true;
  for (const TileVariant& v : k_tiles)
    if (v.lds_bytes > 65536) hipFuncSetAttribute((const void*)v.kernel, hipFuncAttributeMaxDynamicSharedMemorySize, (int)v.lds_bytes);
}

void launch_conv_gemm(const ConvGemmParams& p, int fmt, hipStream_t s) {
  ensure_lds_attrs();
  const TileVariant* v = pick_tile(p, fmt);
  if (v != nullptr && (v->flags & TV_SPLITK) &&
      (p.sk_ws == nullptr || p.sk_cnt == nullptr || ((p.Cin >> 5) % p.splitk) != 0 || (p.Cin >> 5) / p.splitk < 2))
    throw std::runtime_error("conv_gemm: split-K of the halo kernel needs its workspace and splitk | Cin / 32, >= 2 chunks each");
  if ((v == nullptr || v->family == TILE_GENERIC) && p.mode >= MODE_GN_MISH && (p.L & 15) != 0)
    throw std::runtime_error("conv_gemm: a fused GroupNorm epilogue at L = 8 / 4 exists on the gemm16 tile only (whole 256-row tiles)");
  if (v == nullptr) throw std::runtime_error("conv_gemm: a split GEMM of this shape fits no tile (conv_gemm_supported is the contract)");
  dim3 grid(((p.M + 255) >> 8) * ((p.N + 255) >> 8));
  if (v->family == TILE_C2D_SMALL) grid.x = ((p.M + 63) >> 6) * (p.N >> 6);
  if (v->flags & (TV_SPLITK | TV_C2D)) grid.y = p.splitk > 1 ? p.splitk : 1;
  DN_LAUNCH(v->kernel, grid, dim3(v->block), v->lds_bytes, s, p);
}
```

ditreeonlineplanner_amd/csrc/denoise.h:

```cpp
#pragma once
#include <hip/hip_runtime.h>
#include <stdint.h>

enum { MODE_BIAS = 0, MODE_GN_MISH = 1, MODE_GN_MISH_FILM = 2, MODE_GN_MISH_RES = 3 };

enum { ST_BF16 = 0, ST_F32 = 1, ST_F16 = 2 };
static inline int fmt_make(int st, bool split) { return st | (split ? 4 : 0); }
static inline __host__ __device__ int fmt_st(int f) { return f & 3; }
static inline __host__ __device__ bool fmt_split(int f) { return (f & 4) != 0; }
static inline int fmt_es(int f) { return fmt_st(f) == ST_F32 ? 4 : 2; }

struct ConvGemmParams {
  const void* A;
  int lda;
  int in_Lp;
  int in_stride;
  int in_off;
  int taps, Cin;
  const void* W;
  void* Out;
  int ldc;
  int out_Lp, out_stride, out_off;
  int out_coff;
  int L;
  int M, N;
  const float* bias;
  int mode;
  const float* gamma;
  const float* beta;
  int group_ch;
  float eps;
  const float* film;
  int film_ld, film_off;
  const void* Res;
  int ldres, res_Lp, res_off;
  int out_f32;
  int xcd_strips;
  int c2d, c2_H, c2_W, c2_OW, c2_OHW, c2_stride, c2_pad;
  signed char c2_kh[12], c2_kw[12];
  const void* zero;
  long long a_plane, w_plane, out_plane, res_plane;
  float w_scale;
  int splitk;
  long long slab_stride;
  float* sk_ws;
  int* sk_cnt;
  int* sat;
};

void denoise_set_dry_run(bool on);
bool denoise_dry_run();
void launch_conv_gemm(const ConvGemmParams& p, int fmt, hipStream_t s);
bool conv2d_small_eligible(int fmt);
int conv_gemm_kind(const ConvGemmParams& p, int fmt);
bool conv_gemm_supported(const ConvGemmParams& p, int fmt);
void launch_prep_sample(const float* x, void* A0, int B, int P, int D, int fmt, long long plane, hipStream_t s, int* sat = nullptr);
void launch_time_embed(float t, const float* W1, const float* b1, const float* W2, const float* b2, float* out,
                       hipStream_t s);
void launch_prep_cond(const float* temb, const float* map_emb, int E, int E_ld, const float* cond, int G, void* out, int B,
                      int Kpad, int fmt, long long plane, hipStream_t s, int* sat = nullptr);
struct FlowStep {
  int mode;
  float dt;
  float sb, sa, c0, c1, sigma;
  const float* z;
  long long z_row;
  const int* z_idx;
  int z_row0;
};
void launch_final_proj_flow(const void* Y, int C, int Lp, long long plane, const float* W, const float* bias, int D, float* x,
                            FlowStep fs, const double* act_norm , double* actions, int B, int P, int fmt,
                            hipStream_t s);
void launch_gn1d(void* x, int ld, int Lp, int row_off, int coff, int L, int C, const float* gamma, const float* beta, float eps,
                 int mode, const float* film, int film_ld, int film_off, const void* res, int ldres, int res_Lp, int res_off,
                 int B, int fmt, long long x_plane, long long res_plane, hipStream_t s, int* sat = nullptr);
void launch_encoder_stem(const float* lm, int n, const float* W, const float* gamma, const float* beta, void* out, int B, float eps,
                         int fmt, long long plane, hipStream_t s, int* sat = nullptr);
void launch_gn2d(const float* in, int nslab, long long slab_stride, const float* gamma, const float* beta, const void* res,
                 int relu, void* out, int B, int HW, int C, float eps, int fmt, long long res_plane, long long out_plane,
                 hipStream_t s, int* sat = nullptr);
void launch_avgpool2d(const void* in, void* out, int B, int HW, int C, int fmt, long long in_plane, long long out_plane,
                      hipStream_t s);
void launch_unpack_act(const void* in, int ld, int coff, int Lp, int roff, float* out, int B, int L, int C, int fmt,
                       long long plane, hipStream_t s);

enum { ENC_RESNET = 0, ENC_IDENTITY = 1, ENC_MLP = 2, ENC_MAX = 3, ENC_GRID = 4, ENC_CNN = 5 };
struct SmallEncoderParams {
  int kind;
  const float* lm;
  float* out;
  int B, n, E, k;
  const float* w[4];
  const float* b[4];
};
const char* small_encoder_name(int kind);
int small_encoder_width(int kind, int n, int k);
void launch_small_encoder(const SmallEncoderParams& p, hipStream_t s);
```

ditreeonlineplanner_amd/csrc/denoise_plan.hip:

```cpp
#include <algorithm>
#include <cmath>
#include <cstring>
#include <thread>

#include "denoise_state.h"

namespace {

inline uint16_t f2bf_host(float f) {
  uint32_t u;
  std::memcpy(&u, &f, 4);
  if ((u & 0x7fffffffu) > 0x7f800000u) return (uint16_t)((u >> 16) | 0x40);
  u += 0x7fffu + ((u >> 16) & 1u);
  return (uint16_t)(u >> 16);
}
inline float bf2f_host(uint16_t h) {
  uint32_t u = (uint32_t)h << 16;
  float f;
  std::memcpy(&f, &u, 4);
  return f;
}
inline uint16_t f2h_host(float f) { _Float16 h = (_Float16)f; uint16_t u; std::memcpy(&u, &h, 2); return u; }
inline float h2f_host(uint16_t u) { _Float16 h; std::memcpy(&h, &u, 2); return (float)h; }

TapList live_taps(int k, int stride, int pad, int H, int OH) {
  TapList tl{};
  for (int kh = 0; kh < k; ++kh)
    for (int kw = 0; kw < k; ++kw) {
      bool lh = false, lw = false;
      for (int o = 0; o < OH; ++o) {
        const int ih = o * stride + kh - pad, iw = o * stride + kw - pad;
        lh |= (ih >= 0 && ih < H);
        lw |= (iw >= 0 && iw < H);
      }
      if (!(lh && lw)) continue;
      if (tl.n < 12) { tl.kh[tl.n] = (signed char)kh; tl.kw[tl.n] = (signed char)kw; }
      ++tl.n;
    }
  return tl;
}

Act view(const Act& base, int coff, int C) {
  Act v = base;
  v.coff = coff;
  v.C = C;
  return v;
}
Act matrix(void* p, int ld, long long plane = 0) {
  Act a;
  a.p = p; a.C = ld; a.ld = ld; a.padded = false; a.plane = plane;
  return a;
}

}

int* DenoiserState::sat_slot(const std::string& layer, int fmt) {
  if (fmt_st(fmt) != ST_F16 || sat_flags == nullptr) return nullptr;
  for (size_t i = 0; i < sat_names.size(); ++i)
    if (sat_names[i] == layer) return sat_flags + i;
  if ((int)sat_names.size() >= SAT_SLOTS) return sat_flags + SAT_SLOTS - 1;
  sat_names.push_back(layer);
  return sat_flags + sat_names.size() - 1;
}

int DenoiserState::pick_splitk(const ConvGemmParams& p, int fmt) {
  const char* e = getenv("DITREE_DENOISE_SPLITK");
  if (!e || atoi(e) == 0 || !fmt_split(fmt) || p.L == 4 || conv_gemm_kind(p, fmt) != 0) return 1;
  const int tiles = (p.M >> 8) * (p.N >> 8), nvc = p.Cin >> 5;
  int sk = 1;
  static const int cap = [] { const char* c = getenv("DITREE_DENOISE_SPLITK_WGS"); return c ? atoi(c) : 64; }();
  while (sk < 16 && tiles * (sk * 2) <= cap && tiles * (sk * 2) <= SK_MAX_SLABS && nvc % (sk * 2) == 0 && nvc / (sk * 2) >= 2) sk *= 2;
  return sk;
}

void DenoiserState::run_gemm(const ConvGemmParams& p_in, int fmt, hipStream_t s) {
  ConvGemmParams p = p_in;
  p.xcd_strips = 1;
  if (const int sk = pick_splitk(p, fmt); sk > 1) {
    if (sk_ws == nullptr) {
      sk_ws = (float*)dalloc((size_t)SK_MAX_SLABS * 65536 * sizeof(float), false);
      sk_cnt = (int*)dalloc(SK_MAX_SLABS * sizeof(int));
    }
    p.splitk = sk; p.sk_ws = sk_ws; p.sk_cnt = sk_cnt;
  }
  if (!conv_gemm_supported(p, fmt))
    throw std::runtime_error("denoiser layer of shape M " + std::to_string(p.M) + " x N " + std::to_string(p.N) + " x K " +
                             std::to_string(p.taps) + "*" + std::to_string(p.Cin) + " (L " + std::to_string(p.L) +
                             ") fits no tile of this precision");
  prof.launch(p, fmt, s);
}

void* DenoiserState::dalloc(size_t bytes, bool zero) {
  void* p = nullptr;
  if (hipMalloc(&p, bytes ? bytes : 16) != hipSuccess) throw std::runtime_error("hipMalloc failed");
  if (zero && hipMemset(p, 0, bytes ? bytes : 16) != hipSuccess) throw std::runtime_error("hipMemset failed");
  allocs.push_back(p);
  return p;
}
void DenoiserState::free_workspace() {
  for (void* p : allocs) hipFree(p);
  allocs.clear();
  sk_ws = nullptr;
  sk_cnt = nullptr;
  named.clear();
  dev_w.clear();
  dev_f.clear();
  enc_ops.clear();
  unet_ops.clear();
  film_op = nullptr;
  sat_flags = sat_cond = sat_sample = nullptr;
  sat_names.clear();
  prec = -1;
  Bmax = 0;
  Buser = 0;
  temb_t = -1.0f;
}

float* DenoiserState::upload_f32(const std::string& key, const float* src, int64_t n) {
  auto it = dev_f.find(key);
  if (it != dev_f.end()) return it->second;
  float* d = (float*)dalloc((size_t)n * 4, false);
  if (hipMemcpy(d, src, (size_t)n * 4, hipMemcpyHostToDevice) != hipSuccess) throw std::runtime_error("memcpy");
  dev_f[key] = d;
  return d;
}
float* DenoiserState::vec(const std::string& name) {
  const HostParam& hp = P_(name);
  return upload_f32(name, hp.data, hp.n);
}

template <class F>
Packed DenoiserState::pack(const std::string& key, int fmt, int N, int T, int Cin_pad, F get) {
  auto it = dev_w.find(key);
  if (it != dev_w.end()) return it->second;
  const int Npad = (N + 255) / 256 * 256;
  const size_t K = (size_t)T * Cin_pad, total = (size_t)Npad * K;
  const int st = fmt_st(fmt), e = fmt_es(fmt), npl = fmt_split(fmt) ? 2 : 1;
  std::vector<uint8_t> host(total * e * npl, 0);
  const int nthreads = std::max(1u, std::min(16u, std::thread::hardware_concurrency()));
  float mul = 1.0f;
  if (st == ST_F16) {
    std::vector<float> mx(nthreads, 0.0f);
    std::vector<std::thread> th;
    for (int ti = 0; ti < nthreads; ++ti)
      th.emplace_back([&, ti]() {
        float m = 0.f;
        for (int n = ti; n < N; n += nthreads)
          for (int t = 0; t < T; ++t)
            for (int ci = 0; ci < Cin_pad; ++ci) m = std::max(m, std::fabs(get(n, t, ci)));
        mx[ti] = m;
      });
    for (auto& t : th) t.join();
    const float m = *std::max_element(mx.begin(), mx.end());
    if (m > 0.f && std::isfinite(m)) {
      int ex;
      std::frexp(m, &ex);
      mul = std::ldexp(1.0f, 14 - ex);
    }
  }
  std::vector<std::thread> th;
  for (int ti = 0; ti < nthreads; ++ti) {
    th.emplace_back([&, ti]() {
      for (int n = ti; n < N; n += nthreads) {
        for (int t = 0; t < T; ++t)
          for (int ci = 0; ci < Cin_pad; ++ci) {
            const float v = get(n, t, ci) * mul;
            const size_t idx = (size_t)n * K + (size_t)t * Cin_pad + ci;
            if (st == ST_F32) { ((float*)host.data())[idx] = v; continue; }
            uint16_t* hi = (uint16_t*)host.data();
            uint16_t* lo = hi + total;
            if (st == ST_BF16) {
              hi[idx] = f2bf_host(v);
              if (npl == 2) lo[idx] = f2bf_host(v - bf2f_host(hi[idx]));
            } else {
              hi[idx] = f2h_host(v);
              if (npl == 2) lo[idx] = f2h_host(v - h2f_host(hi[idx]));
            }
          }
      }
    });
  }
  for (auto& t : th) t.join();
  Packed pk;
  pk.p = dalloc(total * e * npl, false);
  pk.plane = npl == 2 ? (long long)(total * e) : 0;
  pk.scale = 1.0f / mul;
  if (hipMemcpy(pk.p, host.data(), total * e * npl, hipMemcpyHostToDevice) != hipSuccess) throw std::runtime_error("memcpy");
  dev_w[key] = pk;
  return pk;
}

Act DenoiserState::make_act(const std::string& name, int L, int C, bool padded, int fmt, int rows) {
  Act a;
  a.L = L; a.C = C; a.ld = C; a.coff = 0; a.padded = padded; a.fmt = fmt;
  const size_t bytes = (size_t)rows * a.Lp() * C * fmt_es(fmt);
  const int npl = fmt_split(fmt) ? 2 : 1;
  a.plane = npl == 2 ? (long long)bytes : 0;
  if (npl == 2 && bytes >= 0x7f000000ull) throw std::runtime_error("activation plane of 2 GiB or more: lower the reserved batch");
  a.p = dalloc(bytes * npl);
  named[name] = a;
  return a;
}
Act DenoiserState::make_act(const std::string& name, int L, int C, bool padded) { return make_act(name, L, C, padded, ufmt, Bmax); }

ConvGemmParams DenoiserState::gemm_params(const Act& in, const Act& out, const Packed& wp, int taps, int Cin, int Cout, int in_stride,
                                          int in_off, int out_stride, int out_off, int L, const float* bias, int* sat) {
  ConvGemmParams p{};
  p.A = aptr(in); p.lda = in.ld; p.in_Lp = in.Lp(); p.in_stride = in_stride; p.in_off = in_off; p.taps = taps; p.Cin = Cin;
  p.W = wp.p; p.w_plane = wp.plane; p.w_scale = wp.scale;
  p.a_plane = in.plane; p.out_plane = out.plane;
  p.sat = sat;
  p.Out = (void*)aptr(out); p.ldc = out.ld; p.out_Lp = out.Lp(); p.out_stride = out_stride; p.out_off = out_off;
  p.L = L; p.N = Cout; p.bias = bias; p.mode = MODE_BIAS;
  return p;
}
ConvGemmParams DenoiserState::gemm_params(const Act& in, const Act& out, const Packed& wp, int taps, int Cin, int Cout, int in_stride,
                                          int in_off, int out_stride, int out_off, int L, const std::string& wname) {
  int* sat = sat_slot(wname, ufmt);
  return gemm_params(in, out, wp, taps, Cin, Cout, in_stride, in_off, out_stride, out_off, L, vec(wname + ".bias"), sat);
}
void DenoiserState::set_epilogue(ConvGemmParams& p, int mode, const std::string& gn, int film_off, const Act* res) {
  p.mode = mode; p.eps = 1e-5f;
  if (mode >= MODE_GN_MISH) {
    p.gamma = vec(gn + ".weight"); p.beta = vec(gn + ".bias"); p.group_ch = p.N / 8;
  }
  if (mode == MODE_GN_MISH_FILM) { p.film = film; p.film_ld = film_cols; p.film_off = film_off; }
  if (mode == MODE_GN_MISH_RES) {
    p.Res = aptr(*res); p.ldres = res->ld; p.res_Lp = res->Lp(); p.res_off = res->padded ? 1 : 0; p.res_plane = res->plane;
  }
}
void DenoiserState::push_gemm(const ConvGemmParams& p_in) {
  const int uf = ufmt;
  unet_ops.push_back([this, p = p_in, uf](int, int Bp, hipStream_t s) mutable {
    p.M = Bp * p.L;
    run_gemm(p, uf, s);
  });
}
void DenoiserState::run_rows(ConvGemmParams p, int rows, bool whole_tiles, int fmt, hipStream_t s) {
  const int Mr = whole_tiles ? (rows + 255) / 256 * 256 : rows;
  p.M = Mr; p.L = Mr; p.in_Lp = Mr; p.out_Lp = Mr;
  run_gemm(p, fmt, s);
}
void DenoiserState::add_conv3(const std::string& wname, const Act& in, const Act& out, int mode, const std::string& gn, int film_off,
                              const Act* res) {
  const HostParam& w = P_(wname + ".weight");
  const int Cout = (int)w.dims[0], Cin = (int)w.dims[1];
  const float* wd = w.data;
  const Packed wp = pack(wname, ufmt, Cout, 3, Cin, [=](int n, int t, int ci) { return wd[((size_t)n * Cin + ci) * 3 + t]; });
  ConvGemmParams p = gemm_params(in, out, wp, 3, Cin, Cout, 1, 0, 1, 1, in.L, wname);
  set_epilogue(p, mode, gn, film_off, res);
  emit_block(p, out);
}
void DenoiserState::emit_block(const ConvGemmParams& p, const Act& out) {
  const int Cout = p.N, L = p.L, uf = ufmt;
  const int gch = Cout / 8;
  const bool short_fusable = (L == 8 || L == 4) && fmt_st(uf) != ST_F32;
  const bool fused = p.mode < MODE_GN_MISH ||
                     ((Cout & 255) == 0 && (gch == 64 || gch == 128 || gch == 256) && ((L & 15) == 0 || short_fusable));
  const bool fused_needs_tiles = fused && p.mode >= MODE_GN_MISH && (L & 15) != 0;
  ConvGemmParams qf = p, q = p;
  q.mode = MODE_BIAS;
  unet_ops.push_back([=, this](int, int Bp, hipStream_t s) mutable {
    if (fused && (!fused_needs_tiles || ((Bp * L) & 255) == 0)) {
      qf.M = Bp * L;
      run_gemm(qf, uf, s);
      return;
    }
    q.M = Bp * L;
    run_gemm(q, uf, s);
    prof.note_other();
    launch_gn1d(out.p, out.ld, out.Lp(), 1, out.coff, L, Cout, qf.gamma, qf.beta, 1e-5f, qf.mode, qf.film, qf.film_ld, qf.film_off,
                qf.Res, qf.ldres, qf.res_Lp, qf.res_off, Bp, uf, out.plane, qf.res_plane, s, qf.sat);
  });
}
void DenoiserState::add_conv1(const std::string& wname, const Act& in, const Act& out) {
  const HostParam& w = P_(wname + ".weight");
  const int Cout = (int)w.dims[0], Cin = (int)w.dims[1];
  const float* wd = w.data;
  const Packed wp = pack(wname, ufmt, Cout, 1, Cin, [=](int n, int, int ci) { return wd[(size_t)n * Cin + ci]; });
  push_gemm(gemm_params(in, out, wp, 1, Cin, Cout, 1, 1, 1, 1, in.L, wname));
}
void DenoiserState::add_down(const std::string& wname, const Act& in, const Act& out) {
  const HostParam& w = P_(wname + ".weight");
  const int Cout = (int)w.dims[0], Cin = (int)w.dims[1];
  const float* wd = w.data;
  const Packed wp = pack(wname, ufmt, Cout, 3, Cin, [=](int n, int t, int ci) { return wd[((size_t)n * Cin + ci) * 3 + t]; });
  push_gemm(gemm_params(in, out, wp, 3, Cin, Cout, 2, 0, 1, 1, out.L, wname));
}
void DenoiserState::add_up(const std::string& wname, const Act& in, const Act& out) {
  const HostParam& w = P_(wname + ".weight");
  const int Cin = (int)w.dims[0], Cout = (int)w.dims[1];
  const float* wd = w.data;
  for (int par = 0; par < 2; ++par) {
    const int k0 = par == 0 ? 3 : 2, k1 = par == 0 ? 1 : 0;
    const Packed wp = pack(wname + (par ? ".odd" : ".even"), ufmt, Cout, 2, Cin, [=](int n, int t, int ci) {
      return wd[((size_t)ci * Cout + n) * 4 + (t == 0 ? k0 : k1)];
    });
    push_gemm(gemm_params(in, out, wp, 2, Cin, Cout, 1, par, 2, 1 + par, in.L, wname));
  }
}

void DenoiserState::add_crb(const std::string& pre, const Act& in, const Act& out, int& film_cursor, const std::string& tag) {
  const int Cout = (int)P_(pre + ".blocks.0.block.0.weight").dims[0];
  Act h = make_act(tag + ".h", in.L, Cout);
  const int film_off = film_cursor;
  film_cursor += 2 * Cout;
  add_conv3(pre + ".blocks.0.block.0", in, h, MODE_GN_MISH_FILM, pre + ".blocks.0.block.1", film_off, nullptr);
  Act res = in;
  if (has(pre + ".residual_conv.weight")) {
    res = make_act(tag + ".res", in.L, Cout);
    add_conv1(pre + ".residual_conv", in, res);
  }
  add_conv3(pre + ".blocks.1.block.0", h, out, MODE_GN_MISH_RES, pre + ".blocks.1.block.1", 0, &res);
}

void DenoiserState::build(int prec_, int Bmax_) {
  free_workspace();
  prec = prec_;
  switch (prec) {
    case DITREE_PREC_BF16: ufmt = fmt_make(ST_BF16, false); efmt = ST_BF16; break;
    case DITREE_PREC_F32: ufmt = fmt_make(ST_F32, false); efmt = ST_F32; break;
    case DITREE_PREC_F16X3: ufmt = fmt_make(ST_F16, true); efmt = ufmt; break;
    case DITREE_PREC_BF16X3: ufmt = fmt_make(ST_BF16, true); efmt = ufmt; break;
    case DITREE_PREC_F16: ufmt = fmt_make(ST_F16, false); efmt = ST_F16; break;
    default: throw std::runtime_error("unknown precision");
  }
  prof.ufmt = ufmt;
  sat_flags = (int*)dalloc(SAT_SLOTS * sizeof(int));
  sat_cond = sat_slot("cond_encoder input: Mish(time | map embedding | observation)", ufmt);
  sat_sample = sat_slot("sample (the noisy action sequence)", ufmt);
  const int C0 = dims[0], C1 = dims[1], C2 = dims[2];
  const int L0 = P, L1 = P / 2, L2 = P / 4;
  if (P % 16 != 0 || P < 16 || P > 256 || (256 % P) != 0) throw std::runtime_error("pred_horizon must be 16, 32, 64, 128 or 256");
  bgran = fmt_st(ufmt) != ST_F32 ? std::max(16, 1024 / P) : 16;
  Buser = Bmax_;
  Bmax = (Bmax_ + bgran - 1) / bgran * bgran;
  {
    const long long per_sample = std::max({(long long)(L2 + 2) * 2 * C2, (long long)(L1 + 2) * 2 * C1, (long long)(L0 + 2) * C0,
                                           (long long)L0 * 64}) * fmt_es(ufmt);
    long long cap = std::min<long long>(8192, 0x7f000000LL / per_sample);
    cap = cap / 256 * 256;
    if (cap < 256) throw std::runtime_error("denoiser too large for one 256-sample work unit");
    if (Bmax > cap) Bmax = (int)cap;
  }
  if (fmt_split(ufmt) && ((C0 | C1 | C2) & 255) != 0)
    throw std::runtime_error("the split precisions need down_dims that are multiples of 256 (halo / gemm16 tiles)");
  x_cur = (float*)dalloc((size_t)Bmax * P * D * 4);
  temb = (float*)dalloc(256 * 4);
  condK = (cond_dim + 63) / 64 * 64;
  E_ld = (enc_kind == ENC_RESNET && fmt_split(efmt)) ? (E + 255) / 256 * 256 : E;
  map_emb = (float*)dalloc((size_t)Brows() * E_ld * 4);
  cond_plane = planes() == 2 ? (long long)Brows() * condK * es() : 0;
  condA = dalloc((size_t)Brows() * condK * es() * planes());
  build_film();
  build_unet();
  if (enc_kind != ENC_RESNET) build_encoder_small();
  else build_encoder_resnet();
  if (hipDeviceSynchronize() != hipSuccess) throw std::runtime_error("sync after build failed");
  validate_plan();
}

void DenoiserState::build_film() {
  std::vector<std::string> crbs = {"unet.down_modules.0.0", "unet.down_modules.0.1", "unet.down_modules.1.0",
                                   "unet.down_modules.1.1", "unet.down_modules.2.0", "unet.down_modules.2.1",
                                   "unet.mid_modules.0",    "unet.mid_modules.1",    "unet.up_modules.0.0",
                                   "unet.up_modules.0.1",   "unet.up_modules.1.0",   "unet.up_modules.1.1"};
  std::vector<const float*> wsrc, bsrc;
  std::vector<int> rows, start;
  film_cols = 0;
  for (auto& c : crbs) {
    wsrc.push_back(P_(c + ".cond_encoder.1.weight").data);
    bsrc.push_back(P_(c + ".cond_encoder.1.bias").data);
    rows.push_back((int)P_(c + ".cond_encoder.1.weight").dims[0]);
    start.push_back(film_cols);
    film_cols += rows.back();
  }
  film = (float*)dalloc((size_t)Brows() * film_cols * 4);
  const int cd = cond_dim;
  const Packed wp = pack("film.all", ufmt, film_cols, 1, condK, [=](int n, int, int ci) {
    size_t i = std::upper_bound(start.begin(), start.end(), n) - start.begin() - 1;
    return ci < cd ? wsrc[i][(size_t)(n - start[i]) * cd + ci] : 0.0f;
  });
  std::vector<float> ball(film_cols);
  for (size_t i = 0; i < rows.size(); ++i) std::memcpy(ball.data() + start[i], bsrc[i], (size_t)rows[i] * 4);
  float* bd = upload_f32("film.bias", ball.data(), film_cols);
  ConvGemmParams p = gemm_params(matrix(condA, condK, cond_plane), matrix(film, film_cols), wp, 1, condK, film_cols, 1, 0, 1, 0, 0, bd,
                                 nullptr);
  p.out_f32 = 1;
  const int uf = ufmt;
  film_op = [this, p, uf](int, int Bp, hipStream_t s) { run_rows(p, Bp, fmt_st(uf) != ST_F32, uf, s); };
}

void DenoiserState::build_unet() {
  const int C0 = dims[0], C1 = dims[1], C2 = dims[2];
  const int L0 = P, L1 = P / 2, L2 = P / 4;
  Act a0 = make_act("a0", L0, 64, false);
  const std::string pre = "unet.down_modules.0.0";
  int fc = (int)P_(pre + ".cond_encoder.1.weight").dims[0];
  {
    const float* wd = P_(pre + ".blocks.0.block.0.weight").data;
    const int Dd = D;
    const Packed wp = pack(pre + ".blocks.0.block.0", ufmt, C0, 1, 64, [=](int n, int, int ci) {
      if (ci >= 3 * Dd) return 0.0f;
      const int t = ci / Dd, d = ci - t * Dd;
      return wd[((size_t)n * Dd + d) * 3 + t];
    });
    Act h = make_act("d0b1.h", L0, C0);
    ConvGemmParams p = gemm_params(a0, h, wp, 1, 64, C0, 1, 0, 1, 1, L0, pre + ".blocks.0.block.0");
    set_epilogue(p, MODE_GN_MISH_FILM, pre + ".blocks.0.block.1", 0, nullptr);
    emit_block(p, h);
    const float* wrd = P_(pre + ".residual_conv.weight").data;
    const Packed wrp = pack(pre + ".residual_conv", ufmt, C0, 1, 64, [=](int n, int, int ci) {
      return (ci >= Dd && ci < 2 * Dd) ? wrd[(size_t)n * Dd + (ci - Dd)] : 0.0f;
    });
    Act res = make_act("d0b1.res", L0, C0);
    push_gemm(gemm_params(a0, res, wrp, 1, 64, C0, 1, 0, 1, 1, L0, pre + ".residual_conv"));
    Act o = make_act("d0b1.out", L0, C0);
    add_conv3(pre + ".blocks.1.block.0", h, o, MODE_GN_MISH_RES, pre + ".blocks.1.block.1", 0, &res);
  }
  Act cat1 = make_act("cat1", L1, 2 * C1);
  Act cat0 = make_act("cat0", L2, 2 * C2);
  Act d0o = named["d0b1.out"];
  Act skip0 = make_act("skip0", L0, C0);
  add_crb("unet.down_modules.0.1", d0o, skip0, fc, "d0b2");
  Act d1in = make_act("d1.in", L1, C0);
  add_down("unet.down_modules.0.2.conv", skip0, d1in);
  Act d1o = make_act("d1b1.out", L1, C1);
  add_crb("unet.down_modules.1.0", d1in, d1o, fc, "d1b1");
  Act skip1 = view(cat1, C1, C1);
  named["skip1"] = skip1;
  add_crb("unet.down_modules.1.1", d1o, skip1, fc, "d1b2");
  Act d2in = make_act("d2.in", L2, C1);
  add_down("unet.down_modules.1.2.conv", skip1, d2in);
  Act d2o = make_act("d2b1.out", L2, C2);
  add_crb("unet.down_modules.2.0", d2in, d2o, fc, "d2b1");
  Act skip2 = view(cat0, C2, C2);
  named["skip2"] = skip2;
  add_crb("unet.down_modules.2.1", d2o, skip2, fc, "d2b2");
  Act m1 = make_act("mid1.out", L2, C2);
  add_crb("unet.mid_modules.0", skip2, m1, fc, "mid1");
  Act m2 = view(cat0, 0, C2);
  named["mid2.out"] = m2;
  add_crb("unet.mid_modules.1", m1, m2, fc, "mid2");
  Act u0a = make_act("u0b1.out", L2, C1);
  add_crb("unet.up_modules.0.0", cat0, u0a, fc, "u0b1");
  Act u0b = make_act("u0b2.out", L2, C1);
  add_crb("unet.up_modules.0.1", u0a, u0b, fc, "u0b2");
  Act up0 = view(cat1, 0, C1);
  named["up0.out"] = up0;
  add_up("unet.up_modules.0.2.conv", u0b, up0);
  Act u1a = make_act("u1b1.out", L1, C0);
  add_crb("unet.up_modules.1.0", cat1, u1a, fc, "u1b1");
  Act u1b = make_act("u1b2.out", L1, C0);
  add_crb("unet.up_modules.1.1", u1a, u1b, fc, "u1b2");
  Act fin = make_act("final.in", L0, C0);
  add_up("unet.up_modules.1.2.conv", u1b, fin);
  final_h = make_act("final.h", L0, C0);
  add_conv3("unet.final_conv.0.block.0", fin, final_h, MODE_GN_MISH, "unet.final_conv.0.block.1", 0, nullptr);
  vec("unet.final_conv.1.weight");
  vec("unet.final_conv.1.bias");
  vec("unet.diffusion_step_encoder.1.weight");
  vec("unet.diffusion_step_encoder.1.bias");
  vec("unet.diffusion_step_encoder.3.weight");
  vec("unet.diffusion_step_encoder.3.bias");
}

void DenoiserState::build_encoder_small() {
  SmallEncoderParams q{};
  q.kind = enc_kind; q.n = lm; q.E = E; q.k = enc_k;
  auto transposed = [&](const std::string& name, int out_f, int in_f) {
    const HostParam& w = P_(name);
    if (w.dims.size() != 2 || w.dims[0] != out_f || w.dims[1] != in_f)
      throw std::runtime_error(name + " must be (" + std::to_string(out_f) + ", " + std::to_string(in_f) + ")");
    std::vector<float> t((size_t)out_f * in_f);
    for (int o = 0; o < out_f; ++o)
      for (int i = 0; i < in_f; ++i) t[(size_t)i * out_f + o] = w.data[(size_t)o * in_f + i];
    return upload_f32(name + "#t", t.data(), (int64_t)t.size());
  };
  auto conv_w = [&](const std::string& name, int co, int ci) {
    const HostParam& w = P_(name + ".weight");
    const HostParam& b = P_(name + ".bias");
    if (w.dims.size() != 4 || w.dims[0] != co || w.dims[1] != ci || w.dims[2] != 3 || w.dims[3] != 3 || b.n != co)
      throw std::runtime_error(name + " must be a Conv2d(" + std::to_string(ci) + ", " + std::to_string(co) + ", 3)");
  };
  if (enc_kind == ENC_MLP) {
    const int in_f = lm * lm;
    q.w[0] = transposed("encoder.fc1.weight", 128, in_f);
    q.w[1] = transposed("encoder.fc2.weight", 256, 128);
    q.w[2] = transposed("encoder.fc3.weight", E, 256);
    const int outs[3] = {128, 256, E};
    for (int l = 0; l < 3; ++l) {
      const std::string bn = "encoder.fc" + std::to_string(l + 1) + ".bias";
      if (P_(bn).n != outs[l]) throw std::runtime_error(bn + " must have " + std::to_string(outs[l]) + " elements");
      q.b[l] = vec(bn);
    }
  } else if (enc_kind == ENC_GRID || enc_kind == ENC_CNN) {
    const bool g = enc_kind == ENC_GRID;
    const int nl = g ? 3 : 4;
    const int ci[4] = {1, g ? 3 : 2, g ? 6 : 4, 4}, co[4] = {g ? 3 : 2, g ? 6 : 4, 4, 4};
    for (int l = 0; l < nl; ++l) {
      const std::string nm = "encoder.conv" + std::to_string(l + 1);
      conv_w(nm, co[l], ci[l]);
      q.w[l] = vec(nm + ".weight");
      q.b[l] = vec(nm + ".bias");
    }
  }
  q.out = map_emb;
  enc_ops.push_back([this, q](int B, int, hipStream_t s) {
    prof.note_other();
    SmallEncoderParams r = q;
    r.lm = lm_ptr; r.B = B;
    launch_small_encoder(r, s);
  });
}

void DenoiserState::build_encoder_resnet() {
  const std::string R = "encoder.resnet18.";
  const int pr = efmt;
  const void* zero_row = dalloc(256);
  const size_t gout_per_sample = 9216;
  float* gout = (float*)dalloc((size_t)Bmax * gout_per_sample * 4);
  auto ebuf = [&](const std::string& name, int HW, int C) { return make_act(name, HW, C, false, efmt, HW == 1 ? Brows() : Bmax); };
  auto conv2d = [&](const std::string& wname, const Act& in, int H, int Cout, int k, int stride, int pad, int OH) {
    const HostParam& w = P_(wname + ".weight");
    const float* wd = w.data;
    const int Cw = (int)w.dims[1], Cin = in.C;
    const TapList tl = live_taps(k, stride, pad, H, OH);
    if (Cin % 64 != 0 || tl.n > 12)
      throw std::runtime_error("encoder conv " + wname + " (" + std::to_string(Cin) + " input channels, " + std::to_string(tl.n) +
                               " live taps) fits no implicit-GEMM tile: channels in multiples of 64, at most 12 taps");
    const int K = tl.n * Cin;
    if ((size_t)OH * OH * Cout > gout_per_sample) throw std::runtime_error("encoder scratch region too small for " + wname);
    const Packed wp = pack(wname, efmt, Cout, 1, K, [=](int n, int, int kk) {
      const int c = kk % Cin, t = kk / Cin, kw = tl.kw[t], kh = tl.kh[t];
      return wd[(((size_t)n * Cw + c) * k + kh) * k + kw];
    });
    ConvGemmParams p = gemm_params(in, matrix(gout, Cout), wp, tl.n, Cin, Cout, 1, 0, 1, 0, 0, nullptr, nullptr);
    p.out_f32 = 1;
    p.c2d = 1; p.c2_H = H; p.c2_W = H; p.c2_OW = OH; p.c2_OHW = OH * OH; p.c2_stride = stride; p.c2_pad = pad;
    for (int t = 0; t < tl.n; ++t) { p.c2_kh[t] = tl.kh[t]; p.c2_kw[t] = tl.kw[t]; }
    p.zero = zero_row;
    const int nk_total = tl.n * (Cin / 64);
    const bool small = conv2d_small_eligible(pr);
    const int tiles = small ? ((1024 * OH * OH + 63) / 64) * (Cout / 64) : ((1024 * OH * OH + 255) / 256) * ((Cout + 255) / 256);
    int sk = std::max(1, std::min(std::min(8, nk_total / 2), (small ? 768 : 256) / tiles));
    while (sk > 1 && (size_t)sk * OH * OH * Cout > gout_per_sample) --sk;
    if (sk > 1) {
      const int per = (nk_total + sk - 1) / sk;
      sk = (nk_total + per - 1) / per;
    }
    p.splitk = sk;
    enc_ops.push_back([this, p, pr, OHW = OH * OH](int B, int, hipStream_t s) mutable {
      const int M = B * OHW;
      p.M = M; p.L = M; p.in_Lp = M; p.out_Lp = M;
      p.slab_stride = (long long)M * p.N;
      run_gemm(p, pr, s);
    });
    return sk;
  };
  auto gn = [&](const std::string& gname, int splitk, const Act& out, const Act* res, bool relu) {
    float* ga = vec(gname + ".weight");
    float* be = vec(gname + ".bias");
    const void* rp = res ? res->p : nullptr;
    const int HW = out.L, C = out.C;
    const long long rpl = res ? res->plane : 0;
    {
      const int pp = (C >= 64 && C <= 1024 && (C & (C - 1)) == 0) ? 256 / (C >> 2) : 0;
      if (pp == 0 || (HW + pp - 1) / pp > 7)
        throw std::runtime_error("encoder GroupNorm: unsupported map (" + std::to_string(HW) + " pixels x " + std::to_string(C) + " channels)");
    }
    int* gsat = sat_slot(gname, efmt);
    enc_ops.push_back([=, this](int B, int, hipStream_t s) {
      prof.note_other();
      launch_gn2d(gout, splitk, (long long)B * HW * C, ga, be, rp, relu ? 1 : 0, out.p, B, HW, C, 1e-5f, pr, rpl, out.plane, s, gsat);
    });
  };
  const int H0 = lm;
  auto osz = [](int h, int k, int s, int p) { return (h + 2 * p - k) / s + 1; };
  const int H2 = osz(osz(H0, 7, 2, 3), 3, 2, 1);
  Act pool = ebuf("enc.pool", H2 * H2, 64);
  {
    const HostParam& w = P_(R + "conv1.weight");
    const int Cw = (int)w.dims[1];
    std::vector<float> wf(64 * 49);
    for (int n = 0; n < 64; ++n)
      for (int t = 0; t < 49; ++t) {
        float sacc = 0.f;
        for (int cc = 0; cc < Cw; ++cc) sacc += w.data[((size_t)n * Cw + cc) * 49 + t];
        wf[t * 64 + n] = sacc;
      }
    float* wdev = upload_f32(R + "conv1.weight#folded", wf.data(), 64 * 49);
    float* ga = vec(R + "bn1.weight");
    float* be = vec(R + "bn1.bias");
    int* ssat = sat_slot(R + "conv1", efmt);
    enc_ops.push_back([=, this](int B, int, hipStream_t s) {
      prof.note_other();
      launch_encoder_stem(lm_ptr, H0, wdev, ga, be, pool.p, B, 1e-5f, pr, pool.plane, s, ssat);
    });
  }
  Act cur = pool;
  int Hc = H2;
  const int chans[4] = {64, 128, 256, 512};
  for (int li = 0; li < 4; ++li) {
    for (int bi = 0; bi < 2; ++bi) {
      const std::string pre = R + "layer" + std::to_string(li + 1) + "." + std::to_string(bi);
      const int Cout = chans[li];
      const int stride = (bi == 0 && li > 0) ? 2 : 1;
      const int Ho = osz(Hc, 3, stride, 1);
      const std::string tag = "enc.l" + std::to_string(li + 1) + "." + std::to_string(bi);
      Act t1 = ebuf(tag + ".t", Ho * Ho, Cout);
      gn(pre + ".bn1", conv2d(pre + ".conv1", cur, Hc, Cout, 3, stride, 1, Ho), t1, nullptr, true);
      Act idt = cur;
      if (has(pre + ".downsample.0.weight")) {
        Act ds = ebuf(tag + ".ds", Ho * Ho, Cout);
        gn(pre + ".downsample.1", conv2d(pre + ".downsample.0", cur, Hc, Cout, 1, stride, 0, Ho), ds, nullptr, false);
        idt = ds;
      }
      Act o = ebuf(tag + ".out", Ho * Ho, Cout);
      gn(pre + ".bn2", conv2d(pre + ".conv2", t1, Ho, Cout, 3, 1, 1, Ho), o, &idt, true);
      cur = o;
      Hc = Ho;
    }
  }
  Act pooled = ebuf("enc.avg", 1, cur.C);
  enc_ops.push_back([=, this](int B, int, hipStream_t s) {
    prof.note_other();
    launch_avgpool2d(cur.p, pooled.p, B, cur.L, cur.C, pr, cur.plane, pooled.plane, s);
  });
  {
    const HostParam& w = P_(R + "fc.weight");
    const float* wd = w.data;
    const int Kf = (int)w.dims[1], Nf = (int)w.dims[0];
    const Packed wp = pack(R + "fc", efmt, Nf, 1, Kf, [=](int n, int, int ci) { return wd[(size_t)n * Kf + ci]; });
    const bool esplit = fmt_split(efmt);
    float* bd;
    if (esplit) {
      std::vector<float> bpad(E_ld, 0.0f);
      std::memcpy(bpad.data(), P_(R + "fc.bias").data, (size_t)Nf * 4);
      bd = upload_f32(R + "fc.bias#padded", bpad.data(), E_ld);
    } else {
      bd = vec(R + "fc.bias");
    }
    ConvGemmParams p = gemm_params(matrix(pooled.p, Kf, pooled.plane), matrix(map_emb, E_ld), wp, 1, Kf, esplit ? E_ld : Nf, 1, 0, 1, 0,
                                   0, bd, nullptr);
    p.out_f32 = 1;
    enc_ops.push_back([this, p, pr, esplit](int B, int, hipStream_t s) { run_rows(p, B, esplit, pr, s); });
  }
}

void DenoiserState::validate_plan() {
  float* lm_dev = (float*)dalloc((size_t)bgran * lm * lm * 4);
  lm_ptr = lm_dev;
  denoise_set_dry_run(true);
  try {
    for (auto& op : enc_ops) op(bgran, bgran, nullptr);
    film_op(bgran, bgran, nullptr);
    for (auto& op : unet_ops) op(bgran, bgran, nullptr);
  } catch (...) {
    denoise_set_dry_run(false);
    lm_ptr = nullptr;
    throw;
  }
  denoise_set_dry_run(false);
  lm_ptr = nullptr;
}
```

ditreeonlineplanner_amd/csrc/denoise_prof.h:

```cpp
#pragma once
#include <vector>

#include "denoise.h"

struct DenoiseProfiler {
  bool on = false;
  int mode = 0;
  int ufmt = 0;
  double ms_done[3] = {0, 0, 0};
  int64_t launches_done[3] = {0, 0, 0};
  double flops_done[3] = {0, 0, 0};

  ~DenoiseProfiler() {
    for (auto e : ev) hipEventDestroy(e);
  }
  void set(int enable) {
    collect();
    on = enable != 0;
    mode = enable;
    if (enable) for (int k = 0; k < 3; ++k) { ms_done[k] = 0.0; launches_done[k] = 0; flops_done[k] = 0.0; }
  }
  void note_other() { close_run(); chain = false; }
  void launch(const ConvGemmParams& p, int fmt, hipStream_t s) {
    if (!on) { launch_conv_gemm(p, fmt, s); return; }
    if (used + 2 > ev.size()) {
      const size_t old = ev.size();
      ev.resize(old + 4096);
      for (size_t i = old; i < ev.size(); ++i) hipEventCreate(&ev[i]);
    }
    const double fl = 2.0 * (double)p.M * (double)p.N * (double)p.taps * (double)p.Cin;
    if (mode == 2) {
      const int dom = fmt_st(ufmt) == ST_F32 ? 1 : 0;
      if (conv_gemm_kind(p, fmt) != dom || fmt != ufmt) { close_run(); launch_conv_gemm(p, fmt, s); return; }
      if (run_open && last_stream == s) {
        launch_conv_gemm(p, fmt, s);
        pairs.back().flops += fl;
        pairs.back().launches += 1;
        return;
      }
      close_run();
      const size_t st = used++;
      run_end = used++;
      hipEventRecord(ev[st], s);
      launch_conv_gemm(p, fmt, s);
      pairs.push_back(Rec{st, run_end, dom, fl, 1});
      run_open = true;
      last_stream = s;
      return;
    }
    size_t start;
    if (chain && last_stream == s && used > 0) {
      start = used - 1;
    } else {
      start = used++;
      hipEventRecord(ev[start], s);
    }
    launch_conv_gemm(p, fmt, s);
    const size_t end = used++;
    hipEventRecord(ev[end], s);
    pairs.push_back(Rec{start, end, conv_gemm_kind(p, fmt), fl, 1});
    chain = true;
    last_stream = s;
  }
  void collect() {
    close_run();
    if (used == 0) return;
    hipDeviceSynchronize();
    for (auto& pr : pairs) {
      float ms = 0.f;
      if (hipEventElapsedTime(&ms, ev[pr.a], ev[pr.b]) == hipSuccess) ms_done[pr.kind] += ms;
      launches_done[pr.kind] += pr.launches;
      flops_done[pr.kind] += pr.flops;
    }
    pairs.clear();
    used = 0;
    chain = false;
  }

 private:
  struct Rec { size_t a, b; int kind; double flops; int launches; };
  std::vector<hipEvent_t> ev;
  size_t used = 0;
  std::vector<Rec> pairs;
  bool run_open = false;
  size_t run_end = 0;
  hipStream_t last_stream = nullptr;
  bool chain = false;
  void close_run() {
    if (run_open) { hipEventRecord(ev[run_end], last_stream); run_open = false; }
  }
};
```

ditreeonlineplanner_amd/csrc/denoise_state.h:

```cpp
#pragma once
#include <functional>
#include <map>
#include <stdexcept>
#include <string>
#include <vector>

#include "denoise.h"
#include "denoise_prof.h"
#include "ditree_internal.h"

struct HostParam {
  std::vector<int64_t> dims;
  const float* data = nullptr;
  int64_t n = 0;
};

struct Act {
  void* p = nullptr;
  int L = 0, C = 0;
  int ld = 0, coff = 0;
  bool padded = true;
  long long plane = 0;
  int fmt = 0;
  int Lp() const { return padded ? L + 2 : L; }
};

struct Packed {
  void* p = nullptr;
  long long plane = 0;
  float scale = 1.0f;
};

struct TapList {
  int n;
  signed char kh[12], kw[12];
};

struct DenoiserState {
  using Op = std::function<void(int, int, hipStream_t)>;
  ditree_ctx* ctx = nullptr;
  std::vector<float> blob;
  std::map<std::string, HostParam> params;
  int D = 2, P = 64, E = 400, G = 7, cond_dim = 663, lm = 20;
  int enc_kind = ENC_RESNET;
  int enc_E = -1;
  int enc_k = 0;
  int dims[3] = {512, 1024, 2048};
  bool loaded = false;
  const float* ddpm_coef = nullptr;
  const float* ddpm_z = nullptr;
  long long ddpm_z_row = 0, ddpm_z_step = 0;
  int ddpm_row0 = 0;
  int prec = -1, Bmax = 0;
  int Buser = 0;
  int bgran = 16;
  int ufmt = 0, efmt = 0;
  std::vector<void*> allocs;
  std::map<std::string, Act> named;
  std::map<std::string, Packed> dev_w;
  std::map<std::string, float*> dev_f;
  std::vector<Op> unet_ops, enc_ops;
  Op film_op;
  float* x_cur = nullptr;
  float* temb = nullptr;
  float temb_t = -1.0f;
  float* map_emb = nullptr;
  int E_ld = 400;
  float* film = nullptr;
  void* condA = nullptr;
  long long cond_plane = 0;
  int condK = 0, film_cols = 0;
  Act final_h;
  const float* lm_ptr = nullptr;
  static constexpr int SAT_SLOTS = 256;
  int* sat_flags = nullptr;
  int *sat_cond = nullptr, *sat_sample = nullptr;
  std::vector<std::string> sat_names;
  DenoiseProfiler prof;
  float* sk_ws = nullptr;
  int* sk_cnt = nullptr;
  static constexpr int SK_MAX_SLABS = 512;

  int es() const { return fmt_es(ufmt); }
  int planes() const { return fmt_split(ufmt) ? 2 : 1; }
  int Brows() const { return (Bmax + 255) / 256 * 256; }
  const HostParam& P_(const std::string& name) const {
    auto it = params.find(name);
    if (it == params.end()) throw std::runtime_error("missing parameter " + name);
    return it->second;
  }
  bool has(const std::string& name) const { return params.count(name) != 0; }

  void build(int prec_, int Bmax_);
  void free_workspace();
  void run_gemm(const ConvGemmParams& p_in, int fmt, hipStream_t s);

 private:
  int* sat_slot(const std::string& layer, int fmt);
  int pick_splitk(const ConvGemmParams& p, int fmt);
  void* dalloc(size_t bytes, bool zero = true);
  float* upload_f32(const std::string& key, const float* src, int64_t n);
  float* vec(const std::string& name);
  template <class F>
  Packed pack(const std::string& key, int fmt, int N, int T, int Cin_pad, F get);
  Act make_act(const std::string& name, int L, int C, bool padded, int fmt, int rows);
  Act make_act(const std::string& name, int L, int C, bool padded = true);
  const char* aptr(const Act& a) const { return (const char*)a.p + (size_t)a.coff * es(); }
  ConvGemmParams gemm_params(const Act& in, const Act& out, const Packed& wp, int taps, int Cin, int Cout, int in_stride, int in_off,
                             int out_stride, int out_off, int L, const float* bias, int* sat);
  ConvGemmParams gemm_params(const Act& in, const Act& out, const Packed& wp, int taps, int Cin, int Cout, int in_stride, int in_off,
                             int out_stride, int out_off, int L, const std::string& wname);
  void set_epilogue(ConvGemmParams& p, int mode, const std::string& gn, int film_off, const Act* res);
  void run_rows(ConvGemmParams p, int rows, bool whole_tiles, int fmt, hipStream_t s);
  void push_gemm(const ConvGemmParams& p_in);
  void emit_block(const ConvGemmParams& p, const Act& out);
  void add_conv3(const std::string& wname, const Act& in, const Act& out, int mode, const std::string& gn, int film_off,
                 const Act* res);
  void add_conv1(const std::string& wname, const Act& in, const Act& out);
  void add_down(const std::string& wname, const Act& in, const Act& out);
  void add_up(const std::string& wname, const Act& in, const Act& out);
  void add_crb(const std::string& pre, const Act& in, const Act& out, int& film_cursor, const std::string& tag);
  void build_film();
  void build_unet();
  void build_encoder_small();
  void build_encoder_resnet();
  void validate_plan();
};
```

Measured before the change: 19400 candidate expansions/s.

## Fuse residual 1x1 conv into conv3 halo kernel epilogue as second GEMM

Adds a RES2 variant of the halo16 conv3 kernel. After computing GN+Mish, it keeps the result in the accumulators and runs the residual 1x1 conv GEMM on top of them, then writes a single output. This removes the separate residual GEMM launch and the write and read of the intermediate residual buffer. It is enabled by default for split formats when shapes fit and split-K is not selected. In exchange the kernel gets longer, more complex and heavier on registers, and the fused path cannot use split-K.

```diff
diff --git a/ditreeonlineplanner_amd/csrc/conv_tiles.hip b/ditreeonlineplanner_amd/csrc/conv_tiles.hip
--- a/ditreeonlineplanner_amd/csrc/conv_tiles.hip
+++ b/ditreeonlineplanner_amd/csrc/conv_tiles.hip
@@ -458,21 +458,23 @@
   gemm_epilogue<PREC>(p, acc, smem, tm, tn, tid, lane, r5, h, wm, wn, out_extra);
 }
 
-template <int ET, bool SPLIT, bool SHORT = false>
+struct NoStage { __device__ __forceinline__ void operator()() const {} };
+template <int ET, bool SPLIT, bool SHORT = false, int R2 = 0, class Stage = NoStage>
 __device__ __forceinline__ void gemm_epilogue16(const ConvGemmParams& p, f32x4_t (&acc)[4][8], char* smem, int tm, int tn,
-                                                int tid, int lane, int r4, int h4, int wm, int wn) {
+                                                int tid, int lane, int r4, int h4, int wm, int wn, Stage stage = Stage{}) {
   const int c_l = wn * 128 + 8 * r4;
   const int n0 = tn * 256 + c_l;
   {
+    const float* const bias = R2 == 2 ? p.bias2 : p.bias;
     f32x4_t b0 = {0.f, 0.f, 0.f, 0.f}, b1 = b0;
-    if (p.bias != nullptr) { b0 = *(const f32x4_t*)(p.bias + n0); b1 = *(const f32x4_t*)(p.bias + n0 + 4); }
+    if (bias != nullptr) { b0 = *(const f32x4_t*)(bias + n0); b1 = *(const f32x4_t*)(bias + n0 + 4); }
     if constexpr (ET == 1) {
-      const float ws = p.w_scale;
+      const float ws = R2 == 2 ? p.w_scale2 : p.w_scale;
 #pragma unroll
       for (int mb = 0; mb < 4; ++mb)
 #pragma unroll
         for (int j = 0; j < 4; ++j) { acc[mb][j] = acc[mb][j] * ws + b0[j]; acc[mb][4 + j] = acc[mb][4 + j] * ws + b1[j]; }
-    } else if (p.bias != nullptr) {
+    } else if (bias != nullptr) {
 #pragma unroll
       for (int mb = 0; mb < 4; ++mb)
 #pragma unroll
@@ -520,8 +522,9 @@
     const long long orow = (long long)(blk_b[mb] + lane_b) * p.out_Lp + (long long)(blk_l[mb] + 4 * h4 + lane_l) * p.out_stride + p.out_off;
     return (char*)p.Out + (orow * p.ldc + p.out_coff + n0) * esize;
   };
-  if (p.mode < MODE_GN_MISH) {
-    const int esize = p.out_f32 ? 4 : 2;
+  if (R2 == 2 || (R2 == 0 && p.mode < MODE_GN_MISH)) {
+    const bool out_f32 = R2 == 2 ? false : p.out_f32 != 0;
+    const int esize = out_f32 ? 4 : 2;
     const long long ostep = (long long)p.out_stride * p.ldc * esize;
 #pragma unroll
     for (int mb = 0; mb < 4; ++mb) {
@@ -531,7 +534,7 @@
         float v[8];
 #pragma unroll
         for (int j = 0; j < 8; ++j) v[j] = acc[mb][j][i];
-        if (p.out_f32) {
+        if (out_f32) {
           *(f32x4_t*)ob = f32x4_t{v[0], v[1], v[2], v[3]};
           *(f32x4_t*)(ob + 16) = f32x4_t{v[4], v[5], v[6], v[7]};
         } else {
@@ -541,7 +544,7 @@
     }
     return;
   }
-  const bool has_film = p.mode == MODE_GN_MISH_FILM, has_res = p.mode == MODE_GN_MISH_RES;
+  const bool has_film = R2 == 0 && p.mode == MODE_GN_MISH_FILM, has_res = R2 == 0 && p.mode == MODE_GN_MISH_RES;
   const int spt = 256 / p.L;
   const int ns = spt > 16 ? spt * 4 : 64;
   float* s_sum = (float*)smem;
@@ -575,6 +578,7 @@
     if constexpr (SPLIT) rl[r & 1] = *(const f32x4_t*)(rp + p.res_plane);
   };
   if (has_res) { fetch_res(0); fetch_res(1); }
+  stage();
   __syncthreads();
   const int gi = c_l / p.group_ch;
   const bool wide = p.group_ch >= 128;
@@ -697,6 +701,7 @@
     for (int mb = 0; mb < 4; ++mb) rstd_[mb] = rsqrtf(s[mb] * inv_cnt + p.eps);
   }
   const long long ostep = (long long)p.out_stride * p.ldc * 2;
+  const float inv_ws2 = (R2 == 1 && ET == 1) ? p.inv_w_scale2 : 1.0f;
 #pragma unroll
   for (int mb = 0; mb < 4; ++mb) {
     float mean = mean_[mb];
@@ -724,11 +729,24 @@
 #pragma unroll
       for (int j = 0; j < 4; ++j) { fs[j] = f0[j]; fs[4 + j] = f1[j]; fb[j] = f2[j]; fb[4 + j] = f3[j]; }
     }
-    char* ob = out_ptr(mb, 2);
+    char* ob = R2 == 1 ? nullptr : out_ptr(mb, 2);
 #pragma unroll
     for (int ip = 0; ip < 2; ++ip, ob += 2 * ostep) {
       const int r = mb * 4 + 2 * ip;
       f32x2_t v[8];
+      if constexpr (R2 == 1) {
+#pragma unroll
+        for (int j = 0; j < 8; ++j) {
+          f32x2_t x = pair(mb, j, ip);
+          if constexpr (SPLIT) x = (x - mean) * ga[j] + be[j];
+          else x = x * ga[j] + be[j];
+          x = mish2<SPLIT ? 2 : 0>(x);
+          if constexpr (ET == 1) x = x * inv_ws2;
+          acc[mb][j][2 * ip] = x[0]; acc[mb][j][2 * ip + 1] = x[1];
+        }
+        __builtin_amdgcn_sched_barrier(0);
+        continue;
+      }
       if (has_res) {
         const short8_t h0 = __builtin_bit_cast(short8_t, rh[0]), h1 = __builtin_bit_cast(short8_t, rh[1]);
 #pragma unroll
@@ -764,6 +782,188 @@
       store_row(ob + ostep, row);
       __builtin_amdgcn_sched_barrier(0);
     }
+  }
+}
+
+struct G16Src {
+  __amdgpu_buffer_rsrc_t a_rsrc, w_rsrc;
+  unsigned pae, pao, pbe, pbo;
+  int aq[4], wq[4];
+  int tap_bytes;
+};
+__device__ __forceinline__ void gemm16_src(G16Src& g, const void* A, int lda, int in_Lp, int in_stride, int in_off, int L, unsigned a_plane,
+                                           const void* W, long long K, unsigned w_plane, int tm, int tn, int w, int lane) {
+  long long a_tile0;
+  {
+    const int m0 = tm * 256;
+    const int b0 = m0 / L, l0 = m0 - b0 * L;
+    a_tile0 = (((long long)b0 * in_Lp + (long long)l0 * in_stride + in_off) * lda) * 2;
+  }
+  g.a_rsrc = __builtin_amdgcn_make_buffer_rsrc((void*)((const char*)A + a_tile0), 0, 0x7fffffff, 0x00020000);
+  g.w_rsrc = __builtin_amdgcn_make_buffer_rsrc((void*)((const char*)W + ((long long)tn * 256) * K * 2), 0, 0x7fffffff, 0x00020000);
+  unsigned pae, pao, pbe, pbo;
+  {
+    const int lr = lane >> 3;
+    const int slot0 = (lane & 7) ^ (lr >> 1), slot1 = slot0 ^ 4;
+    const int lrb = lr / L, lro = lrb * in_Lp + (lr - lrb * L) * in_stride;
+    pae = (unsigned)((lro * lda + (slot0 & 3) * 8) * 2) + ((slot0 & 4) ? a_plane : 0u);
+    pao = (unsigned)((lro * lda + (slot1 & 3) * 8) * 2) + ((slot1 & 4) ? a_plane : 0u);
+    pbe = (unsigned)(((long long)(8 * lr) * K + (slot0 & 3) * 8) * 2) + ((slot0 & 4) ? w_plane : 0u);
+    pbo = (unsigned)(((long long)(8 * lr) * K + (slot1 & 3) * 8) * 2) + ((slot1 & 4) ? w_plane : 0u);
+#pragma unroll
+    for (int q = 0; q < 4; ++q) {
+      const int r0 = (w * 4 + q) * 8;
+      const int m = tm * 256 + r0;
+      const int b = m / L, l = m - b * L;
+      g.aq[q] = (int)((((long long)b * in_Lp + (long long)l * in_stride + in_off) * lda) * 2 - a_tile0);
+      const int cu = (r0 & 128) + 8 * (r0 & 8) + ((r0 >> 4) & 7);
+      g.wq[q] = (int)((long long)cu * K * 2);
+    }
+  }
+  g.tap_bytes = lda * 2;
+  g.pae = pae; g.pao = pao; g.pbe = pbe; g.pbo = pbo;
+}
+template <int ET>
+__device__ __forceinline__ void gemm16_walk(char* smem, f32x4_t (&acc)[4][8], const G16Src& g, int nc, int nk, int w, int r4, int h4, int wm,
+                                            int wn) {
+  constexpr int BUF = 32768, W_BASE = 2 * BUF;
+  constexpr int KB = 64;
+  const __amdgpu_buffer_rsrc_t a_rsrc = g.a_rsrc, w_rsrc = g.w_rsrc;
+  const unsigned pae = g.pae, pao = g.pao, pbe = g.pbe, pbo = g.pbo;
+  const int (&aq)[4] = g.aq;
+  const int (&wq)[4] = g.wq;
+  const int tap_bytes = g.tap_bytes;
+  auto src_off = [&](int k, int& ao, int& wo) {
+    const int t = k / nc, c = k - t * nc;
+    ao = t * tap_bytes + c * KB;
+    wo = k * KB;
+  };
+  auto issue_wq = [&](int kv, int q) {
+    int ao, wo;
+    src_off(kv, ao, wo);
+    __builtin_amdgcn_raw_ptr_buffer_load_lds(w_rsrc, (LDS_AS void*)(smem + W_BASE + (kv & 1) * BUF + (w * 4 + q) * 1024), 16,
+                                             (q & 1) ? pbo : pbe, wq[q] + wo, 0, 0);
+  };
+  const int a_row = wm * 64 + r4;
+  const int swa = (a_row >> 1) & 7;
+  const int a_off = a_row * 128, b_off = (wn * 128 + r4) * 128;
+  const int swb = (r4 >> 1) & 7;
+  short8_t af[2][4], bq[2][4];
+  auto rdA = [&](int set, int k, int ks) {
+    const char* ab = smem + (k & 1) * BUF + a_off + ((((ks << 2) | h4) ^ swa) << 4);
+#pragma unroll
+    for (int mb = 0; mb < 4; ++mb) af[set][mb] = *(const short8_t*)(ab + mb * 2048);
+  };
+  auto rdB = [&](int set, int k, int ks, int half) {
+    const char* wb = smem + W_BASE + (k & 1) * BUF + b_off + half * 8192 + ((((ks << 2) | h4) ^ swb) << 4);
+#pragma unroll
+    for (int jj = 0; jj < 4; ++jj) bq[set][jj] = *(const short8_t*)(wb + jj * 2048);
+  };
+  auto mm = [&](int aset, int bset, int half, int mb, int jj) {
+    acc[mb][half * 4 + jj] = mfma16<ET>(af[aset][mb], bq[bset][jj], acc[mb][half * 4 + jj]);
+  };
+  auto mm16 = [&](int aset, int bset, int half) {
+#pragma unroll
+    for (int mb = 0; mb < 4; ++mb)
+#pragma unroll
+      for (int jj = 0; jj < 4; ++jj) mm(aset, bset, half, mb, (mb & 1) ? 3 - jj : jj);
+  };
+  auto step = [&](auto tNext, auto tIssue, int k) {
+    constexpr bool HAS_NEXT = decltype(tNext)::value, ISSUE = decltype(tIssue)::value;
+    rdB(1, k, 1, 1);
+    mm16(0, 0, 0);
+    if constexpr (HAS_NEXT) {
+      issue_wq(k + 1, 0); issue_wq(k + 1, 1);
+      __builtin_amdgcn_sched_group_barrier(0x100, 4, 0);
+      __builtin_amdgcn_sched_group_barrier(0x008, 4, 0);
+      __builtin_amdgcn_sched_group_barrier(0x020, 1, 0);
+      __builtin_amdgcn_sched_group_barrier(0x008, 4, 0);
+      __builtin_amdgcn_sched_group_barrier(0x020, 1, 0);
+      __builtin_amdgcn_sched_group_barrier(0x008, 8, 0);
+    } else {
+      __builtin_amdgcn_sched_group_barrier(0x100, 4, 0);
+      __builtin_amdgcn_sched_group_barrier(0x008, 16, 0);
+    }
+    __builtin_amdgcn_sched_barrier(0);
+    rdB(0, k, 0, 0);
+    rdA(1, k, 1);
+    mm16(0, 1, 1);
+    if constexpr (HAS_NEXT) {
+      issue_wq(k + 1, 2); issue_wq(k + 1, 3);
+      __builtin_amdgcn_sched_group_barrier(0x100, 8, 0);
+      __builtin_amdgcn_sched_group_barrier(0x008, 4, 0);
+      __builtin_amdgcn_sched_group_barrier(0x020, 1, 0);
+      __builtin_amdgcn_sched_group_barrier(0x008, 4, 0);
+      __builtin_amdgcn_sched_group_barrier(0x020, 1, 0);
+      __builtin_amdgcn_sched_group_barrier(0x008, 8, 0);
+    } else {
+      __builtin_amdgcn_sched_group_barrier(0x100, 8, 0);
+      __builtin_amdgcn_sched_group_barrier(0x008, 16, 0);
+    }
+    __builtin_amdgcn_sched_barrier(0);
+    rdB(1, k, 0, 1);
+    mm16(0, 0, 0);
+    __builtin_amdgcn_sched_group_barrier(0x100, 4, 0);
+    __builtin_amdgcn_sched_group_barrier(0x008, 16, 0);
+    __builtin_amdgcn_sched_barrier(0);
+    mm16(1, 0, 0);
+    __builtin_amdgcn_sched_barrier(0);
+    mm16(0, 1, 1);
+    __builtin_amdgcn_sched_barrier(0);
+    int ao2 = 0, wo2 = 0;
+    if constexpr (ISSUE) src_off(k + 2, ao2, wo2);
+    if constexpr (HAS_NEXT) {
+      asm volatile("s_waitcnt vmcnt(0) lgkmcnt(0)" ::: "memory");
+      __builtin_amdgcn_s_barrier();
+      rdA(0, k + 1, 0);
+      rdB(0, k + 1, 1, 0);
+    }
+#pragma unroll
+    for (int mb = 0; mb < 4; ++mb)
+#pragma unroll
+      for (int jj = 0; jj < 4; ++jj) {
+        mm(1, 1, 1, mb, (mb & 1) ? 3 - jj : jj);
+        if constexpr (ISSUE) {
+          const int m = mb * 4 + jj, i = (m & 1) ? -1 : (m >> 1);
+          if (i >= 0 && i < 4)
+            __builtin_amdgcn_raw_ptr_buffer_load_lds(a_rsrc, (LDS_AS void*)(smem + (k & 1) * BUF + (w * 4 + i) * 1024), 16,
+                                                     (i & 1) ? pao : pae, aq[i] + ao2, 0, 0);
+        }
+      }
+    if constexpr (HAS_NEXT) __builtin_amdgcn_sched_group_barrier(0x100, 8, 1);
+#pragma unroll
+    for (int i = 0; i < 16; ++i) {
+      __builtin_amdgcn_sched_group_barrier(0x008, 1, 1);
+      if (ISSUE && !(i & 1) && i < 8) __builtin_amdgcn_sched_group_barrier(0x020, 1, 1);
+    }
+    __builtin_amdgcn_sched_barrier(0);
+  };
+  using Tt = std::true_type;
+  using Ff = std::false_type;
+
+  asm volatile("s_waitcnt vmcnt(0)" ::: "memory");
+  __builtin_amdgcn_s_barrier();
+  rdA(0, 0, 0);
+  rdB(0, 0, 1, 0);
+  for (int k = 0; k < nk - 2; ++k) step(Tt{}, Tt{}, k);
+  if (nk >= 2) step(Tt{}, Ff{}, nk - 2);
+  step(Ff{}, Ff{}, nk - 1);
+}
+__device__ __forceinline__ void gemm16_stage_first(char* smem, const G16Src& g, int nc, int nk, int w) {
+  constexpr int BUF = 32768, W_BASE = 2 * BUF;
+#pragma unroll
+  for (int q = 0; q < 4; ++q)
+    __builtin_amdgcn_raw_ptr_buffer_load_lds(g.a_rsrc, (LDS_AS void*)(smem + (w * 4 + q) * 1024), 16, (q & 1) ? g.pao : g.pae, g.aq[q], 0, 0);
+#pragma unroll
+  for (int q = 0; q < 4; ++q)
+    __builtin_amdgcn_raw_ptr_buffer_load_lds(g.w_rsrc, (LDS_AS void*)(smem + W_BASE + (w * 4 + q) * 1024), 16, (q & 1) ? g.pbo : g.pbe,
+                                             g.wq[q], 0, 0);
+  if (nk > 1) {
+    const int ao = nc > 1 ? 64 : g.tap_bytes;
+#pragma unroll
+    for (int q = 0; q < 4; ++q)
+      __builtin_amdgcn_raw_ptr_buffer_load_lds(g.a_rsrc, (LDS_AS void*)(smem + BUF + (w * 4 + q) * 1024), 16, (q & 1) ? g.pao : g.pae,
+                                               g.aq[q] + ao, 0, 0);
   }
 }
 
@@ -1006,8 +1206,12 @@
   gemm_epilogue16<ET, false>(p, acc, smem, tm, tn, tid, lane, r4, h4, wm, wn);
 }
 
-template <int ET, bool SHORT = false, bool SPLITK = false, int NP = 5>
+enum { NP_RES2 = 8 };
+template <int ET, bool SHORT = false, bool SPLITK = false, int NPV = 5>
 __global__ void __launch_bounds__(512, 2) conv3_halo16x3_kernel(ConvGemmParams p) {
+  constexpr int NP = NPV & 7;
+  constexpr bool RES2 = (NPV & NP_RES2) != 0;
+  static_assert(!(RES2 && (SPLITK || SHORT || NP != 5)), "the fused residual walk: 16 | L, no split-K form");
   extern __shared__ __attribute__((aligned(16))) char smem[];
   static_assert(NP == 5 || NP == 6, "five or six activation pieces");
   constexpr int A_BUF = NP * 8192, W_BUF = 32768, W_BASE = 2 * A_BUF;
@@ -1275,7 +1479,24 @@
     }
     if (tid == 0) p.sk_cnt[tile] = 0;
   }
-  gemm_epilogue16<ET, true, SHORT>(p, acc, smem, tm, tn, tid, lane, r4, h4, wm, wn);
+  if constexpr (RES2) {
+    const int nk2 = p.Cin2 >> 5;
+    G16Src g2;
+    int lane2 = tid;
+    asm volatile("" : "+v"(lane2));
+    lane2 &= 63;
+    gemm16_src(g2, p.A2, p.lda2, p.in_Lp2, p.in_stride2, p.in_off2, L, (unsigned)p.a_plane2, p.W2, (long long)p.Cin2,
+                     (unsigned)p.w_plane2, tm, tn, w, lane2);
+    char* const scratch = smem + 131072;
+    gemm_epilogue16<ET, true, SHORT, 1>(p, acc, scratch, tm, tn, tid, lane, r4, h4, wm, wn,
+                                        [&]() { gemm16_stage_first(smem, g2, nk2, nk2, w); });
+    int r4w = r4, h4w = h4;
+    asm volatile("" : "+v"(r4w), "+v"(h4w));
+    gemm16_walk<ET>(smem, acc, g2, nk2, nk2, w, r4w, h4w, wm, wn);
+    gemm_epilogue16<ET, true, SHORT, 2>(p, acc, scratch, tm, tn, tid, lane, r4, h4, wm, wn);
+  } else {
+    gemm_epilogue16<ET, true, SHORT>(p, acc, smem, tm, tn, tid, lane, r4, h4, wm, wn);
+  }
 #ifdef HALO16_STAMP
   __syncthreads();
   if (tid == 0) {
@@ -1635,7 +1856,8 @@
        TV_SHORT = 2,
        TV_SPLITK = 4,
        TV_NP6 = 8,
-       TV_C2D = 16 };
+       TV_C2D = 16,
+       TV_RES2 = 32 };
 struct TileVariant {
   void (*kernel)(ConvGemmParams);
   unsigned lds_bytes;
@@ -1657,6 +1879,8 @@
     {conv3_halo16x3_kernel<1, true, true>, 147456, 512, TILE_HALO, ST_F16, TV_SPLIT | TV_SHORT | TV_SPLITK, 0},
     {conv3_halo16x3_kernel<0, true, false, 6>, 163840, 512, TILE_HALO, ST_BF16, TV_SPLIT | TV_SHORT | TV_NP6, 0},
     {conv3_halo16x3_kernel<1, true, false, 6>, 163840, 512, TILE_HALO, ST_F16, TV_SPLIT | TV_SHORT | TV_NP6, 0},
+    {conv3_halo16x3_kernel<0, false, false, 5 + NP_RES2>, 147456, 512, TILE_HALO, ST_BF16, TV_SPLIT | TV_RES2, 0},
+    {conv3_halo16x3_kernel<1, false, false, 5 + NP_RES2>, 147456, 512, TILE_HALO, ST_F16, TV_SPLIT | TV_RES2, 0},
     {gemm16_kernel<0, false>, 131072, 512, TILE_GEMM16, ST_BF16, 0, 1},
     {gemm16_kernel<1, false>, 131072, 512, TILE_GEMM16, ST_F16, 0, 1},
     {gemm16_kernel<0, true>, 131072, 512, TILE_GEMM16, ST_BF16, TV_SPLIT, 1},
@@ -1689,11 +1913,14 @@
   const bool tile16 = st != ST_F32 && !p.c2d && (p.M & 255) == 0 && (p.N & 255) == 0 && (p.Cin & 63) == 0;
   const bool l_ok = p.L >= 16 || (p.L == 8 && split) || (p.L == 4 && split && p.splitk <= 1);
   if (tile16 && p.taps == 3 && p.in_stride == 1 && p.in_Lp == p.L + 2 && (256 % p.L) == 0 && l_ok && p.Cin >= 192) {
+    if (p.mode == MODE_GN_MISH_RES2)
+      return split && p.L >= 16 && p.splitk <= 1 ? find_tile(TILE_HALO, st, TV_SPLIT | TV_RES2) : nullptr;
     if (!split) return find_tile(TILE_HALO, st, 0);
     const unsigned fshort = p.L <= 8 ? TV_SHORT : 0;
     if (p.splitk > 1) return find_tile(TILE_HALO, st, TV_SPLIT | fshort | TV_SPLITK);
     return find_tile(TILE_HALO, st, TV_SPLIT | fshort | (p.L == 4 ? TV_NP6 : 0));
   }
+  if (p.mode == MODE_GN_MISH_RES2) return nullptr;
   const bool short_l = p.L == 8 || p.L == 4;
   if (tile16 && (!p.out_f32 || p.mode == MODE_BIAS) && p.taps >= 1 && p.taps <= 3 && ((p.L & 15) == 0 || short_l) && p.M > 0 &&
       (p.mode == MODE_BIAS || (256 % p.L) == 0))
@@ -1709,6 +1936,11 @@
   return v != nullptr ? v->kind : (p.c2d ? 2 : 1);
 }
 bool conv_gemm_supported(const ConvGemmParams& p, int fmt) { return pick_tile(p, fmt) != nullptr; }
+bool conv_gemm_res2_fusable(int fmt, int L, int Cin, int Cout, int Cin2) {
+  const int gch = Cout / 8;
+  return fmt_split(fmt) && L >= 16 && (256 % L) == 0 && (Cout & 255) == 0 && (gch == 64 || gch == 128 || gch == 256) &&
+         (Cin & 63) == 0 && Cin >= 192 && (Cin2 & 31) == 0 && Cin2 >= 64;
+}
 
 static void ensure_lds_attrs() {
   static bool done[64] = {};
@@ -1728,6 +1960,13 @@
     throw std::runtime_error("conv_gemm: split-K of the halo kernel needs its workspace and splitk | Cin / 32, >= 2 chunks each");
   if ((v == nullptr || v->family == TILE_GENERIC) && p.mode >= MODE_GN_MISH && (p.L & 15) != 0)
     throw std::runtime_error("conv_gemm: a fused GroupNorm epilogue at L = 8 / 4 exists on the gemm16 tile only (whole 256-row tiles)");
+  if (p.mode == MODE_GN_MISH_RES2) {
+    if (v == nullptr || !(v->flags & TV_RES2) || p.A2 == nullptr || p.W2 == nullptr || (p.Cin2 & 31) != 0 || p.Cin2 < 64 ||
+        p.lda2 < p.Cin2 || p.in_Lp2 < p.L || p.in_stride2 < 1 || (256 % p.L) != 0 || p.out_f32 ||
+        p.w_scale2 * p.inv_w_scale2 != 1.0f || p.a_plane2 <= 0 || p.w_plane2 <= 0 || p.a_plane2 >= 0x7f000000LL ||
+        p.w_plane2 >= 0x7f000000LL)
+      throw std::runtime_error("conv_gemm: MODE_GN_MISH_RES2 needs the split halo tile at 16 | L and a complete second operand set");
+  }
   if (v == nullptr) throw std::runtime_error("conv_gemm: a split GEMM of this shape fits no tile (conv_gemm_supported is the contract)");
   dim3 grid(((p.M + 255) >> 8) * ((p.N + 255) >> 8));
   if (v->family == TILE_C2D_SMALL) grid.x = ((p.M + 63) >> 6) * (p.N >> 6);
diff --git a/ditreeonlineplanner_amd/csrc/denoise.h b/ditreeonlineplanner_amd/csrc/denoise.h
--- a/ditreeonlineplanner_amd/csrc/denoise.h
+++ b/ditreeonlineplanner_amd/csrc/denoise.h
@@ -2,7 +2,7 @@
 #include <hip/hip_runtime.h>
 #include <stdint.h>
 
-enum { MODE_BIAS = 0, MODE_GN_MISH = 1, MODE_GN_MISH_FILM = 2, MODE_GN_MISH_RES = 3 };
+enum { MODE_BIAS = 0, MODE_GN_MISH = 1, MODE_GN_MISH_FILM = 2, MODE_GN_MISH_RES = 3, MODE_GN_MISH_RES2 = 4 };
 
 enum { ST_BF16 = 0, ST_F32 = 1, ST_F16 = 2 };
 static inline int fmt_make(int st, bool split) { return st | (split ? 4 : 0); }
@@ -46,6 +46,13 @@
   float* sk_ws;
   int* sk_cnt;
   int* sat;
+  const void* A2;
+  const void* W2;
+  const float* bias2;
+  long long a_plane2, w_plane2;
+  int lda2, in_Lp2, in_stride2, in_off2;
+  int Cin2;
+  float w_scale2, inv_w_scale2;
 };
 
 void denoise_set_dry_run(bool on);
@@ -54,6 +61,7 @@
 bool conv2d_small_eligible(int fmt);
 int conv_gemm_kind(const ConvGemmParams& p, int fmt);
 bool conv_gemm_supported(const ConvGemmParams& p, int fmt);
+bool conv_gemm_res2_fusable(int fmt, int L, int Cin, int Cout, int Cin2);
 void launch_prep_sample(const float* x, void* A0, int B, int P, int D, int fmt, long long plane, hipStream_t s, int* sat = nullptr);
 void launch_time_embed(float t, const float* W1, const float* b1, const float* W2, const float* b2, float* out,
                        hipStream_t s);
diff --git a/ditreeonlineplanner_amd/csrc/denoise_plan.hip b/ditreeonlineplanner_amd/csrc/denoise_plan.hip
--- a/ditreeonlineplanner_amd/csrc/denoise_plan.hip
+++ b/ditreeonlineplanner_amd/csrc/denoise_plan.hip
@@ -66,6 +66,7 @@
 int DenoiserState::pick_splitk(const ConvGemmParams& p, int fmt) {
   const char* e = getenv("DITREE_DENOISE_SPLITK");
   if (!e || atoi(e) == 0 || !fmt_split(fmt) || p.L == 4 || conv_gemm_kind(p, fmt) != 0) return 1;
+  if (p.mode == MODE_GN_MISH_RES2) return 1;
   const int tiles = (p.M >> 8) * (p.N >> 8), nvc = p.Cin >> 5;
   int sk = 1;
   static const int cap = [] { const char* c = getenv("DITREE_DENOISE_SPLITK_WGS"); return c ? atoi(c) : 64; }();
@@ -219,8 +220,15 @@
   int* sat = sat_slot(wname, ufmt);
   return gemm_params(in, out, wp, taps, Cin, Cout, in_stride, in_off, out_stride, out_off, L, vec(wname + ".bias"), sat);
 }
-void DenoiserState::set_epilogue(ConvGemmParams& p, int mode, const std::string& gn, int film_off, const Act* res) {
+void DenoiserState::set_epilogue(ConvGemmParams& p, int mode, const std::string& gn, int film_off, const Act* res, const Res2* r2) {
   p.mode = mode; p.eps = 1e-5f;
+  if (mode == MODE_GN_MISH_RES2) {
+    const Act& a = r2->in;
+    p.A2 = aptr(a); p.lda2 = a.ld; p.in_Lp2 = a.Lp(); p.in_stride2 = 1; p.in_off2 = a.padded ? 1 : 0; p.a_plane2 = a.plane;
+    p.W2 = r2->w.p; p.w_plane2 = r2->w.plane; p.Cin2 = r2->Cin;
+    p.w_scale2 = r2->w.scale; p.inv_w_scale2 = 1.0f / r2->w.scale;
+    p.bias2 = r2->bias;
+  }
   if (mode >= MODE_GN_MISH) {
     p.gamma = vec(gn + ".weight"); p.beta = vec(gn + ".bias"); p.group_ch = p.N / 8;
   }
@@ -241,15 +249,45 @@
   p.M = Mr; p.L = Mr; p.in_Lp = Mr; p.out_Lp = Mr;
   run_gemm(p, fmt, s);
 }
-void DenoiserState::add_conv3(const std::string& wname, const Act& in, const Act& out, int mode, const std::string& gn, int film_off,
-                              const Act* res) {
+ConvGemmParams DenoiserState::conv3_params(const std::string& wname, const Act& in, const Act& out, int mode, const std::string& gn,
+                                           int film_off, const Act* res, const Res2* r2) {
   const HostParam& w = P_(wname + ".weight");
   const int Cout = (int)w.dims[0], Cin = (int)w.dims[1];
   const float* wd = w.data;
   const Packed wp = pack(wname, ufmt, Cout, 3, Cin, [=](int n, int t, int ci) { return wd[((size_t)n * Cin + ci) * 3 + t]; });
   ConvGemmParams p = gemm_params(in, out, wp, 3, Cin, Cout, 1, 0, 1, 1, in.L, wname);
-  set_epilogue(p, mode, gn, film_off, res);
-  emit_block(p, out);
+  set_epilogue(p, mode, gn, film_off, res, r2);
+  return p;
+}
+void DenoiserState::add_conv3(const std::string& wname, const Act& in, const Act& out, int mode, const std::string& gn, int film_off,
+                              const Act* res) {
+  emit_block(conv3_params(wname, in, out, mode, gn, film_off, res, nullptr), out);
+}
+void DenoiserState::emit_res2_block(const std::string& wname, const Act& h, const Act& out, const std::string& gn, const Res2& r2,
+                                    const std::string& tag) {
+  const ConvGemmParams pf = conv3_params(wname, h, out, MODE_GN_MISH_RES2, gn, 0, nullptr, &r2);
+  Act res_proto = out;
+  res_proto.p = nullptr; res_proto.ld = out.C; res_proto.coff = 0; res_proto.padded = true;
+  ConvGemmParams pc = conv3_params(wname, h, out, MODE_GN_MISH_RES, gn, 0, &res_proto, nullptr);
+  ConvGemmParams pr = gemm_params(r2.in, res_proto, r2.w, 1, r2.Cin, out.C, 1, r2.in.padded ? 1 : 0, 1, 1, out.L, r2.bias, pf.sat);
+  const int uf = ufmt, L = out.L, Cout = out.C;
+  unet_ops.push_back([=, this](int, int Bp, hipStream_t s) mutable {
+    pc.M = Bp * L;
+    if (pick_splitk(pc, uf) <= 1) {
+      ConvGemmParams q = pf;
+      q.M = Bp * L;
+      run_gemm(q, uf, s);
+      return;
+    }
+    if (pc.Res == nullptr) {
+      const Act res = make_act(tag + ".res", L, Cout);
+      pc.Res = res.p; pc.res_plane = res.plane;
+      pr.Out = res.p; pr.out_plane = res.plane;
+    }
+    pr.M = Bp * L;
+    run_gemm(pr, uf, s);
+    run_gemm(pc, uf, s);
+  });
 }
 void DenoiserState::emit_block(const ConvGemmParams& p, const Act& out) {
   const int Cout = p.N, L = p.L, uf = ufmt;
@@ -273,12 +311,13 @@
                 qf.Res, qf.ldres, qf.res_Lp, qf.res_off, Bp, uf, out.plane, qf.res_plane, s, qf.sat);
   });
 }
-void DenoiserState::add_conv1(const std::string& wname, const Act& in, const Act& out) {
+DenoiserState::Res2 DenoiserState::add_conv1(const std::string& wname, const Act& in, const Act* out) {
   const HostParam& w = P_(wname + ".weight");
   const int Cout = (int)w.dims[0], Cin = (int)w.dims[1];
   const float* wd = w.data;
   const Packed wp = pack(wname, ufmt, Cout, 1, Cin, [=](int n, int, int ci) { return wd[(size_t)n * Cin + ci]; });
-  push_gemm(gemm_params(in, out, wp, 1, Cin, Cout, 1, 1, 1, 1, in.L, wname));
+  if (out != nullptr) push_gemm(gemm_params(in, *out, wp, 1, Cin, Cout, 1, 1, 1, 1, in.L, wname));
+  return Res2{in, wp, vec(wname + ".bias"), Cin};
 }
 void DenoiserState::add_down(const std::string& wname, const Act& in, const Act& out) {
   const HostParam& w = P_(wname + ".weight");
@@ -308,8 +347,13 @@
   add_conv3(pre + ".blocks.0.block.0", in, h, MODE_GN_MISH_FILM, pre + ".blocks.0.block.1", film_off, nullptr);
   Act res = in;
   if (has(pre + ".residual_conv.weight")) {
+    const int Cin2 = (int)P_(pre + ".residual_conv.weight").dims[1];
+    if (fuse_res && conv_gemm_res2_fusable(ufmt, in.L, Cout, Cout, Cin2)) {
+      emit_res2_block(pre + ".blocks.1.block.0", h, out, pre + ".blocks.1.block.1", add_conv1(pre + ".residual_conv", in, nullptr), tag);
+      return;
+    }
     res = make_act(tag + ".res", in.L, Cout);
-    add_conv1(pre + ".residual_conv", in, res);
+    add_conv1(pre + ".residual_conv", in, &res);
   }
   add_conv3(pre + ".blocks.1.block.0", h, out, MODE_GN_MISH_RES, pre + ".blocks.1.block.1", 0, &res);
 }
@@ -326,6 +370,10 @@
     default: throw std::runtime_error("unknown precision");
   }
   prof.ufmt = ufmt;
+  {
+    const char* fr = getenv("DITREE_FUSE_RES");
+    fuse_res = !(fr != nullptr && atoi(fr) == 0);
+  }
   sat_flags = (int*)dalloc(SAT_SLOTS * sizeof(int));
   sat_cond = sat_slot("cond_encoder input: Mish(time | map embedding | observation)", ufmt);
   sat_sample = sat_slot("sample (the noisy action sequence)", ufmt);
@@ -413,10 +461,14 @@
     const Packed wrp = pack(pre + ".residual_conv", ufmt, C0, 1, 64, [=](int n, int, int ci) {
       return (ci >= Dd && ci < 2 * Dd) ? wrd[(size_t)n * Dd + (ci - Dd)] : 0.0f;
     });
-    Act res = make_act("d0b1.res", L0, C0);
-    push_gemm(gemm_params(a0, res, wrp, 1, 64, C0, 1, 0, 1, 1, L0, pre + ".residual_conv"));
     Act o = make_act("d0b1.out", L0, C0);
-    add_conv3(pre + ".blocks.1.block.0", h, o, MODE_GN_MISH_RES, pre + ".blocks.1.block.1", 0, &res);
+    if (fuse_res && conv_gemm_res2_fusable(ufmt, L0, C0, C0, 64)) {
+      emit_res2_block(pre + ".blocks.1.block.0", h, o, pre + ".blocks.1.block.1", Res2{a0, wrp, vec(pre + ".residual_conv.bias"), 64}, "d0b1");
+    } else {
+      Act res = make_act("d0b1.res", L0, C0);
+      push_gemm(gemm_params(a0, res, wrp, 1, 64, C0, 1, 0, 1, 1, L0, pre + ".residual_conv"));
+      add_conv3(pre + ".blocks.1.block.0", h, o, MODE_GN_MISH_RES, pre + ".blocks.1.block.1", 0, &res);
+    }
   }
   Act cat1 = make_act("cat1", L1, 2 * C1);
   Act cat0 = make_act("cat0", L2, 2 * C2);
diff --git a/ditreeonlineplanner_amd/csrc/denoise_prof.h b/ditreeonlineplanner_amd/csrc/denoise_prof.h
--- a/ditreeonlineplanner_amd/csrc/denoise_prof.h
+++ b/ditreeonlineplanner_amd/csrc/denoise_prof.h
@@ -28,7 +28,7 @@
       ev.resize(old + 4096);
       for (size_t i = old; i < ev.size(); ++i) hipEventCreate(&ev[i]);
     }
-    const double fl = 2.0 * (double)p.M * (double)p.N * (double)p.taps * (double)p.Cin;
+    const double fl = 2.0 * (double)p.M * (double)p.N * ((double)p.taps * (double)p.Cin + (p.mode == MODE_GN_MISH_RES2 ? (double)p.Cin2 : 0.0));
     if (mode == 2) {
       const int dom = fmt_st(ufmt) == ST_F32 ? 1 : 0;
       if (conv_gemm_kind(p, fmt) != dom || fmt != ufmt) { close_run(); launch_conv_gemm(p, fmt, s); return; }
diff --git a/ditreeonlineplanner_amd/csrc/denoise_state.h b/ditreeonlineplanner_amd/csrc/denoise_state.h
--- a/ditreeonlineplanner_amd/csrc/denoise_state.h
+++ b/ditreeonlineplanner_amd/csrc/denoise_state.h
@@ -80,6 +80,13 @@
   float* sk_ws = nullptr;
   int* sk_cnt = nullptr;
   static constexpr int SK_MAX_SLABS = 512;
+  bool fuse_res = true;
+  struct Res2 {
+    Act in;
+    Packed w;
+    const float* bias;
+    int Cin;
+  };
 
   int es() const { return fmt_es(ufmt); }
   int planes() const { return fmt_split(ufmt) ? 2 : 1; }
@@ -110,13 +117,17 @@
                              int out_stride, int out_off, int L, const float* bias, int* sat);
   ConvGemmParams gemm_params(const Act& in, const Act& out, const Packed& wp, int taps, int Cin, int Cout, int in_stride, int in_off,
                              int out_stride, int out_off, int L, const std::string& wname);
-  void set_epilogue(ConvGemmParams& p, int mode, const std::string& gn, int film_off, const Act* res);
+  void set_epilogue(ConvGemmParams& p, int mode, const std::string& gn, int film_off, const Act* res, const Res2* r2 = nullptr);
   void run_rows(ConvGemmParams p, int rows, bool whole_tiles, int fmt, hipStream_t s);
   void push_gemm(const ConvGemmParams& p_in);
   void emit_block(const ConvGemmParams& p, const Act& out);
+  ConvGemmParams conv3_params(const std::string& wname, const Act& in, const Act& out, int mode, const std::string& gn, int film_off,
+                              const Act* res, const Res2* r2);
   void add_conv3(const std::string& wname, const Act& in, const Act& out, int mode, const std::string& gn, int film_off,
                  const Act* res);
-  void add_conv1(const std::string& wname, const Act& in, const Act& out);
+  void emit_res2_block(const std::string& wname, const Act& h, const Act& out, const std::string& gn, const Res2& r2,
+                       const std::string& tag);
+  Res2 add_conv1(const std::string& wname, const Act& in, const Act* out);
   void add_down(const std::string& wname, const Act& in, const Act& out);
   void add_up(const std::string& wname, const Act& in, const Act& out);
   void add_crb(const std::string& pre, const Act& in, const Act& out, int& film_cursor, const std::string& tag);
```

Result: no change. 19580 candidate expansions/s, median of 6 (+1.0%).
